# ccuchengwei/LongReadSelfCorrect

Hardware: AMD Instinct MI355X
Metric: corrected Mbases/s (whole node) (higher is better)
Workload: dtype int64

## Files before the change

longreadselfcorrect_amd/csrc/capi_batch.cpp:

```cpp
#include <cmath>
#include <limits>

#include "capi_internal.h"

using namespace lrsc;

extern "C" void lrsc_batch_destroy(lrsc_batch* b)
{
    if(!b) return;
    if(b->ctx) (void)hipSetDevice(b->ctx->device);
    if(b->d_codes) (void)hipFree(b->d_codes);
    if(b->d_off) (void)hipFree(b->d_off);
    if(b->d_chunk) (void)hipFree(b->d_chunk);
    void* ptrs[] = {b->d_freq, b->d_base_counted, b->d_valid, b->d_flags, b->d_zeros, b->d_attr, b->d_start_bits, b->d_seeds,
                    b->d_seed_count, b->d_thr, b->d_scan_tmp, b->d_outcasts, b->d_outcast_count, b->d_walk_log, b->d_ratio};
    for(void* q : ptrs) if(q) (void)hipFree(q);
    delete b;
}

extern "C" int lrsc_batch_create(lrsc_ctx* ctx, const char* reads, const uint64_t* read_off, uint32_t n_reads,
                                 lrsc_batch** out)
{
    if(!ctx || !out || n_reads == 0) return fail(LRSC_ERR_ARG, "null / empty batch");
    int st = check_offsets(read_off, n_reads);
    if(st != LRSC_OK) return st;
    const uint64_t total = read_off[n_reads];
    if(total == 0 || !reads) return fail(LRSC_ERR_ARG, "empty batch");
    HIP_TRY(hipSetDevice(ctx->device));
    lrsc_batch* b = new(std::nothrow) lrsc_batch();
    if(!b) return fail(LRSC_ERR_NOMEM, "lrsc_batch");
    b->ctx = ctx;
    b->n_reads = n_reads;
    b->total_bases = total;
    const uint64_t n_chunks = (total + (1ull << kChunkShift) - 1) >> kChunkShift;
    hipError_t e = hipMalloc(reinterpret_cast<void**>(&b->d_codes), total);
    if(e == hipSuccess) e = hipMalloc(reinterpret_cast<void**>(&b->d_off), (n_reads + 1) * sizeof(uint64_t));
    if(e == hipSuccess) e = hipMalloc(reinterpret_cast<void**>(&b->d_chunk), n_chunks * sizeof(uint32_t));
    if(e != hipSuccess) { lrsc_batch_destroy(b); return hip_fail(e, "batch alloc"); }
    const uint64_t slice = 256ull << 20;
    for(uint64_t o = 0; o < total; o += slice) {
        const uint64_t n = std::min(slice, total - o);
        st = upload_and_encode(ctx, reads + o, n, b->d_codes + o);
        if(st != LRSC_OK) { lrsc_batch_destroy(b); return st; }
    }
    e = hipMemcpyAsync(b->d_off, read_off, (n_reads + 1) * sizeof(uint64_t), hipMemcpyHostToDevice, ctx->stream);
    if(e == hipSuccess) e = launch_chunk_table(b->d_off, n_reads, total, b->d_chunk, ctx->stream);
    if(e == hipSuccess) e = hipStreamSynchronize(ctx->stream);
    if(e != hipSuccess) { lrsc_batch_destroy(b); return hip_fail(e, "batch upload"); }
    *out = b;
    return LRSC_OK;
}

static uint32_t pool_from_params(const lrsc_params& p, uint8_t* ks)
{
    std::vector<int> v = {5, 9, p.scan_kmer_len};
    for(int i = 0; i < 3; ++i) v.push_back(p.start_kmer_len + p.offset[i]);
    std::sort(v.begin(), v.end());
    v.erase(std::unique(v.begin(), v.end()), v.end());
    uint32_t n = 0;
    for(int x : v) if(x > 0 && x < 256 && n < kMaxPool) ks[n++] = (uint8_t)x;
    return n;
}

static const float kThresholdFormula[3][6] = {
    {0.0004799107143, -0.008037815126, 0.03673552754, 0.1850695903, -1.572552521, 18.0522088},
    {0.0003348214286, -0.009112394958, 0.04286714686, 0.240519958, -1.8793367350, 21.29319228},
    {0.01714285714, -0.6193907563, 2.266956783, 17.28450630, -100.6983493, 1103.571729}};

extern "C" int lrsc_kmer_thresholds_range(int coverage, int end, float* out)
{
    if(!out || end < 15) return fail(LRSC_ERR_ARG, "null table / end < 15");
    const int start = 15, stride = end + 2;
    for(int mode = 0; mode < 3; ++mode) {
        for(int k = 0; k < stride; ++k) out[mode * stride + k] = 0.0f;
        float cavity = std::numeric_limits<float>::max();
        const float* f = kThresholdFormula[mode];
        const int x = coverage;
        for(int y = start; y <= end; ++y) {
            float v = f[0] * x * x + f[1] * x * y + f[2] * y * y + f[3] * x + f[4] * y + f[5];
            v = std::fmax(v, 2.0f);
            cavity = std::fmin(cavity, v);
            out[mode * stride + y] = cavity;
        }
    }
    return LRSC_OK;
}

extern "C" int lrsc_kmer_thresholds(int coverage, float* out)
{
    return lrsc_kmer_thresholds_range(coverage, 50, out);
}

static int batch_setup_rows(lrsc_ctx* ctx, lrsc_batch* b)
{
    if(b->n_k != 0) return LRSC_OK;
    const lrsc_params& p = ctx->params;
    b->n_k = pool_from_params(p, b->ks);
    for(auto& x : b->row_of_k) x = -1;
    for(auto& x : b->freq_index) x = -1;
    int wanted[4] = {p.scan_kmer_len, p.start_kmer_len + p.offset[0], p.start_kmer_len + p.offset[1],
                     p.start_kmer_len + p.offset[2]};
    int min_k = 1 << 30;
    for(int i = 0; i < 4; ++i) {
        const int k = wanted[i];
        if(k <= 0 || k > 51) return fail(LRSC_ERR_ARG, "k-mer sizes must lie in 1..51");
        if(i > 0 && k < min_k) min_k = k;
        if(b->row_of_k[k] >= 0) continue;
        for(uint32_t j = 0; j < b->n_k; ++j)
            if(b->ks[j] == k) { b->freq_index[j] = (int8_t)b->n_rows; b->row_of_k[k] = (int8_t)b->n_rows; ++b->n_rows; }
        if(b->row_of_k[k] < 0) return fail(LRSC_ERR_ARG, "k-mer size missing from the pool");
    }
    b->min_k = (uint32_t)min_k;
    if(b->total_bases >= (1ull << 32)) return fail(LRSC_ERR_UNSUPPORTED, "a resident batch holds < 2^32 bases");
    HIP_TRY(hipMalloc(reinterpret_cast<void**>(&b->d_freq), (size_t)b->n_rows * b->total_bases * sizeof(int32_t)));
    HIP_TRY(hipMalloc(reinterpret_cast<void**>(&b->d_base_counted), b->total_bases));
    HIP_TRY(hipMalloc(reinterpret_cast<void**>(&b->d_valid), b->total_bases));
    return LRSC_OK;
}

static GridArgs batch_grid_args(const lrsc_batch* b)
{
    GridArgs a{};
    a.codes = b->d_codes;
    a.read_off = b->d_off;
    a.chunk_read = b->d_chunk;
    a.total_bases = b->total_bases;
    a.n_reads = b->n_reads;
    a.n_k = b->n_k;
    for(uint32_t i = 0; i < b->n_k; ++i) { a.ks[i] = b->ks[i]; a.freq_index[i] = b->freq_index[i]; }
    a.freq = b->d_freq;
    a.base_counted = b->d_base_counted;
    a.valid_mask = b->d_valid;
    return a;
}

extern "C" int lrsc_batch_kmer_grid(lrsc_ctx* ctx, lrsc_batch* b)
{
    if(!ctx || !b || b->ctx != ctx) return fail(LRSC_ERR_ARG, "batch does not belong to this ctx");
    HIP_TRY(hipSetDevice(ctx->device));
    int st = batch_setup_rows(ctx, b);
    if(st != LRSC_OK) return st;
    const GridArgs a = batch_grid_args(b);
    st = timed_launch(ctx, LRSC_K_GRID, [&]() { return launch_kmer_grid(ctx->fm, a, ctx->d_ctr, ctx->stream); });
    if(st == LRSC_OK) b->grid_done = true;
    return st;
}

static int batch_setup_seeds(lrsc_ctx* ctx, lrsc_batch* b)
{
    if(b->d_seeds) return LRSC_OK;
    b->seed_cap = b->total_bases / b->min_k + b->n_reads + 1;
    HIP_TRY(hipMalloc(reinterpret_cast<void**>(&b->d_flags), b->total_bases * sizeof(unsigned long long)));
    HIP_TRY(hipMalloc(reinterpret_cast<void**>(&b->d_zeros), b->total_bases * sizeof(uint32_t)));
    HIP_TRY(hipMalloc(reinterpret_cast<void**>(&b->d_attr), b->total_bases));
    HIP_TRY(hipMalloc(reinterpret_cast<void**>(&b->d_start_bits), ((b->total_bases + 255) / 256) * 4 * sizeof(unsigned long long)));
    HIP_TRY(hipMalloc(reinterpret_cast<void**>(&b->d_seeds), b->seed_cap * kSeedInts * sizeof(int32_t)));
    HIP_TRY(hipMalloc(reinterpret_cast<void**>(&b->d_seed_count), (size_t)b->n_reads * sizeof(uint32_t)));
    if(b->debug_flags & LRSC_DEBUG_RATIO) HIP_TRY(hipMalloc(reinterpret_cast<void**>(&b->d_ratio), b->total_bases * sizeof(float)));
    if(b->debug_flags & LRSC_DEBUG_OUTCASTS) {
        HIP_TRY(hipMalloc(reinterpret_cast<void**>(&b->d_outcasts), b->seed_cap * kSeedInts * sizeof(int32_t)));
        HIP_TRY(hipMalloc(reinterpret_cast<void**>(&b->d_outcast_count), (size_t)b->n_reads * sizeof(uint32_t)));
    }
    HIP_TRY(hipMalloc(reinterpret_cast<void**>(&b->d_thr), 3 * 52 * sizeof(float)));
    float thr[3 * 52];
    (void)lrsc_kmer_thresholds(ctx->params.pb_coverage, thr);
    HIP_TRY(hipMemcpy(b->d_thr, thr, sizeof(thr), hipMemcpyHostToDevice));
    return LRSC_OK;
}

static SeedArgs batch_seed_args(const lrsc_ctx* ctx, const lrsc_batch* b)
{
    const lrsc_params& p = ctx->params;
    SeedArgs a{};
    a.codes = b->d_codes; a.read_off = b->d_off; a.chunk_read = b->d_chunk;
    a.total_bases = b->total_bases; a.n_reads = b->n_reads;
    a.freq = b->d_freq; a.valid_mask = b->d_valid; a.base_counted = b->d_base_counted;
    for(int i = 0; i < 64; ++i) a.row_of_k[i] = b->row_of_k[i];
    a.base_k = b->ks[0];
    a.start_kmer_len = p.start_kmer_len; a.scan_kmer_len = p.scan_kmer_len; a.kmer_len_up_bound = p.kmer_len_up_bound;
    a.pb_coverage = p.pb_coverage; a.mode = p.mode; a.manual = p.manual; a.radius = p.radius;
    for(int i = 0; i < 3; ++i) a.offset[i] = p.offset[i];
    a.hh_ratio = p.hh_ratio;
    a.thresholds = b->d_thr;
    a.flags = b->d_flags; a.zeros = b->d_zeros; a.attribute = b->d_attr; a.start_bits = b->d_start_bits; a.seeds = b->d_seeds; a.seed_count = b->d_seed_count;
    a.outcasts = b->d_outcasts; a.outcast_count = b->d_outcast_count; a.ratio = b->d_ratio;
    return a;
}

extern "C" int lrsc_batch_find_seeds(lrsc_ctx* ctx, lrsc_batch* b)
{
    if(!ctx || !b || b->ctx != ctx) return fail(LRSC_ERR_ARG, "batch does not belong to this ctx");
    if(ctx->params.kmer_len_up_bound > 50) return fail(LRSC_ERR_ARG, "kmer_len_up_bound must be <= 50 (threshold table)");
    if(ctx->params.manual && (ctx->params.mode < 0 || ctx->params.mode > 2)) return fail(LRSC_ERR_ARG, "mode must be 0, 1 or 2");
    int st = lrsc_batch_kmer_grid(ctx, b);
    if(st != LRSC_OK) return st;
    st = batch_setup_seeds(ctx, b);
    if(st != LRSC_OK) return st;
    const SeedArgs a = batch_seed_args(ctx, b);
    st = timed_launch(ctx, LRSC_K_SEEDS, [&]() {
        hipError_t e = launch_seed_modes(a, ctx->stream);
        if(e == hipSuccess) e = scan_seed_flags(b->d_flags, b->d_zeros, b->total_bases, &b->d_scan_tmp, &b->scan_tmp_cap, ctx->stream);
        if(e == hipSuccess) e = launch_seed_attribute(a, ctx->stream);
        if(e == hipSuccess) e = launch_seed_scan(ctx->fm, a, b->min_k, ctx->d_ctr, ctx->stream);
        return e;
    });
    if(st == LRSC_OK) b->seeds_done = true;
    return st;
}

extern "C" int lrsc_batch_seeds(lrsc_ctx* ctx, lrsc_batch* b, uint32_t* seed_count, lrsc_seed* seeds, uint64_t cap,
                                uint64_t* n_seeds, int8_t* attribute)
{
    if(!ctx || !b || b->ctx != ctx || !seed_count || !n_seeds) return fail(LRSC_ERR_ARG, "null / foreign batch");
    if(!b->seeds_done) return fail(LRSC_ERR_ARG, "call lrsc_batch_find_seeds first");
    HIP_TRY(hipSetDevice(ctx->device));
    HIP_TRY(hipMemcpy(seed_count, b->d_seed_count, (size_t)b->n_reads * sizeof(uint32_t), hipMemcpyDeviceToHost));
    std::vector<uint64_t> off(b->n_reads + 1);
    HIP_TRY(hipMemcpy(off.data(), b->d_off, off.size() * sizeof(uint64_t), hipMemcpyDeviceToHost));
    uint64_t total = 0;
    for(uint32_t r = 0; r < b->n_reads; ++r) total += seed_count[r];
    *n_seeds = total;
    if(total > cap) return fail(LRSC_ERR_CAPACITY, "seed buffer too small");
    if(seeds) {
        static_assert(sizeof(lrsc_seed) == kSeedInts * sizeof(int32_t), "lrsc_seed layout");
        uint64_t w = 0;
        for(uint32_t r = 0; r < b->n_reads; ++r) {
            if(seed_count[r] == 0) continue;
            const uint64_t slab = seed_slab(off[r], r, b->min_k);
            HIP_TRY(hipMemcpy(seeds + w, b->d_seeds + slab * kSeedInts, (size_t)seed_count[r] * sizeof(lrsc_seed),
                              hipMemcpyDeviceToHost));
            w += seed_count[r];
        }
    }
    if(attribute) HIP_TRY(hipMemcpy(attribute, b->d_attr, b->total_bases, hipMemcpyDeviceToHost));
    return LRSC_OK;
}

extern "C" int lrsc_find_seeds(lrsc_ctx* ctx, const char* reads, const uint64_t* read_off, uint32_t n_reads,
                               uint32_t* seed_count, lrsc_seed* seeds, uint64_t cap, uint64_t* n_seeds, int8_t* attribute)
{
    lrsc_batch* b = nullptr;
    int st = lrsc_batch_create(ctx, reads, read_off, n_reads, &b);
    if(st != LRSC_OK) return st;
    st = lrsc_batch_find_seeds(ctx, b);
    if(st == LRSC_OK) st = lrsc_batch_seeds(ctx, b, seed_count, seeds, cap, n_seeds, attribute);
    lrsc_batch_destroy(b);
    return st;
}

extern "C" int lrsc_batch_set_debug(lrsc_batch* b, int flags)
{
    if(!b) return fail(LRSC_ERR_ARG, "null batch");
    if(flags & ~(LRSC_DEBUG_OUTCASTS | LRSC_DEBUG_WALKS | LRSC_DEBUG_RATIO)) return fail(LRSC_ERR_ARG, "unknown debug flag");
    if(b->d_seeds) return fail(LRSC_ERR_ARG, "lrsc_batch_set_debug must precede lrsc_batch_find_seeds");
    b->debug_flags = flags;
    return LRSC_OK;
}

extern "C" int lrsc_batch_outcast_seeds(lrsc_ctx* ctx, lrsc_batch* b, uint32_t* outcast_count, lrsc_seed* seeds, uint64_t cap,
                                        uint64_t* n_seeds)
{
    if(!ctx || !b || b->ctx != ctx || !outcast_count || !n_seeds) return fail(LRSC_ERR_ARG, "null / foreign batch");
    if(!b->seeds_done || !b->d_outcasts) return fail(LRSC_ERR_ARG, "needs LRSC_DEBUG_OUTCASTS and lrsc_batch_find_seeds");
    HIP_TRY(hipSetDevice(ctx->device));
    HIP_TRY(hipMemcpy(outcast_count, b->d_outcast_count, (size_t)b->n_reads * sizeof(uint32_t), hipMemcpyDeviceToHost));
    std::vector<uint64_t> off(b->n_reads + 1);
    HIP_TRY(hipMemcpy(off.data(), b->d_off, off.size() * sizeof(uint64_t), hipMemcpyDeviceToHost));
    uint64_t total = 0;
    for(uint32_t r = 0; r < b->n_reads; ++r) total += outcast_count[r];
    *n_seeds = total;
    if(total > cap) return fail(LRSC_ERR_CAPACITY, "seed buffer too small");
    uint64_t w = 0;
    for(uint32_t r = 0; seeds && r < b->n_reads; ++r) {
        if(outcast_count[r] == 0) continue;
        const uint64_t slab = seed_slab(off[r], r, b->min_k);
        HIP_TRY(hipMemcpy(seeds + w, b->d_outcasts + slab * kSeedInts, (size_t)outcast_count[r] * sizeof(lrsc_seed), hipMemcpyDeviceToHost));
        w += outcast_count[r];
    }
    return LRSC_OK;
}

extern "C" int lrsc_batch_repeat_ratio(lrsc_ctx* ctx, lrsc_batch* b, float* ratio)
{
    if(!ctx || !b || b->ctx != ctx || !ratio) return fail(LRSC_ERR_ARG, "null / foreign batch");
    if(!b->seeds_done || !b->d_ratio) return fail(LRSC_ERR_ARG, "needs LRSC_DEBUG_RATIO and lrsc_batch_find_seeds");
    HIP_TRY(hipSetDevice(ctx->device));
    HIP_TRY(hipMemcpy(ratio, b->d_ratio, b->total_bases * sizeof(float), hipMemcpyDeviceToHost));
    return LRSC_OK;
}

extern "C" int lrsc_batch_walk_log(lrsc_ctx* ctx, lrsc_batch* b, uint8_t* log, uint64_t cap)
{
    if(!ctx || !b || b->ctx != ctx || !log) return fail(LRSC_ERR_ARG, "null / foreign batch");
    if(!b->walk_log_done || !b->d_walk_log) return fail(LRSC_ERR_ARG, "needs LRSC_DEBUG_WALKS and lrsc_batch_correct");
    HIP_TRY(hipSetDevice(ctx->device));
    std::vector<uint32_t> count(b->n_reads);
    std::vector<uint64_t> off(b->n_reads + 1);
    HIP_TRY(hipMemcpy(count.data(), b->d_seed_count, count.size() * sizeof(uint32_t), hipMemcpyDeviceToHost));
    HIP_TRY(hipMemcpy(off.data(), b->d_off, off.size() * sizeof(uint64_t), hipMemcpyDeviceToHost));
    std::vector<uint8_t> all(b->seed_cap);
    HIP_TRY(hipMemcpy(all.data(), b->d_walk_log, b->seed_cap, hipMemcpyDeviceToHost));
    uint64_t w = 0;
    for(uint32_t r = 0; r < b->n_reads; ++r) {
        if(w + count[r] > cap) return fail(LRSC_ERR_CAPACITY, "walk log buffer too small");
        if(count[r]) std::memcpy(log + w, all.data() + seed_slab(off[r], r, b->min_k), count[r]);
        w += count[r];
    }
    return LRSC_OK;
}
```

longreadselfcorrect_amd/csrc/capi_core.cpp:

```cpp
#include <cmath>
#include <limits>

#include "capi_internal.h"

using namespace lrsc;

static thread_local std::string g_last_error;

int lrsc::fail(int status, const std::string& msg)
{
    g_last_error = msg;
    return status;
}
int lrsc::hip_fail(hipError_t e, const char* what)
{
    g_last_error = std::string(what) + ": " + hipGetErrorString(e);
    return LRSC_ERR_DEVICE;
}

extern "C" const char* lrsc_strerror(int status)
{
    switch(status) {
        case LRSC_OK: return "ok";
        case LRSC_ERR_IO: return "I/O error";
        case LRSC_ERR_FORMAT: return "BWT file is not properly formatted";
        case LRSC_ERR_ARG: return "invalid argument";
        case LRSC_ERR_NOMEM: return "out of memory";
        case LRSC_ERR_DEVICE: return "HIP device error";
        case LRSC_ERR_CAPACITY: return "output buffer too small";
        case LRSC_ERR_UNSUPPORTED: return "unsupported";
        case LRSC_ERR_LIMIT: return "internal capacity exceeded";
        default: return "unknown error";
    }
}
extern "C" const char* lrsc_last_error(void) { return g_last_error.c_str(); }
extern "C" int lrsc_abi_version(void) { return LRSC_ABI_VERSION; }

extern "C" int lrsc_params_default(int genome, int coverage, lrsc_params* out)
{
    if(!out) return fail(LRSC_ERR_ARG, "null params");
    int order;
    switch(genome) {
        case 5: order = 0; break;
        case 10: order = 1; break;
        case 100: order = 2; break;
        default: return fail(LRSC_ERR_ARG, "genome must be 5, 10 or 100");
    }
    static const int size[3] = {17, 19, 21};
    std::memset(out, 0, sizeof(*out));
    out->pb_coverage = coverage;
    out->error_rate = 0.15;
    out->start_kmer_len = size[order];
    out->offset[0] = 0;
    out->offset[1] = 2 * std::min(std::max(coverage / 30 - 1, 0), order + 1);
    out->offset[2] = -2 * (order + 1);
    out->mode = 1;
    out->manual = 0;
    out->scan_kmer_len = 19;
    out->kmer_len_up_bound = 50;
    out->radius = 100;
    out->hh_ratio = 0.6f;
    out->next_target = 1;
    out->max_leaves = 32;
    out->idmer_len = 9;
    out->min_kmer_len = 13;
    out->split = 0;
    out->no_dp = 0;
    return LRSC_OK;
}

uint64_t lrsc::env_bytes(const char* name, uint64_t dflt, unsigned shift)
{
    if(const char* e = std::getenv(name)) return std::max<uint64_t>(1, (uint64_t)std::atoll(e)) << shift;
    return dflt;
}

static uint32_t env_clamped(const char* name, uint32_t dflt, int lo, int hi)
{
    if(const char* e = std::getenv(name)) return (uint32_t)std::min(hi, std::max(lo, std::atoi(e)));
    return dflt;
}

uint32_t lrsc::resident_waves(const lrsc_ctx* ctx, uint32_t per_simd)
{
    int cus = 256;
    (void)hipDeviceGetAttribute(&cus, hipDeviceAttributeMultiprocessorCount, ctx->device);
    return (uint32_t)cus * 4u * per_simd;
}

Tunables lrsc::read_tunables(const lrsc_ctx* ctx)
{
    const int kIntMax = std::numeric_limits<int>::max();
    Tunables t;
    t.wp_prep_bytes = env_bytes("LRSC_WP_PREP_MB", 24ull << 30, 20);
    t.wp_lane_bytes = env_bytes("LRSC_WP_LANE_MB", 32ull << 30, 20);
    t.wp_lanes = env_clamped("LRSC_WP_LANES", resident_waves(ctx, 2) * 64u, 64, kIntMax);
    t.wp_gen_quorum = env_clamped("LRSC_WP_GEN_QUORUM", 70, 0, 100);
    t.wp_gen_wait = env_clamped("LRSC_WP_GEN_WAIT", 6, 0, kIntMax);
    t.wp_wide_cap = env_clamped("LRSC_WP_WIDE_CAP", kNarrowLeaves, 1, (int)kNarrowLeaves);
    t.wp_wave = env_clamped("LRSC_WP_WAVE", 1, 0, 2);
    { const char* e = std::getenv("LRSC_WP_BEGIN_SORT"); t.wp_begin_sort = e && e[0] != '0'; }
    t.dp_chunk_bytes = env_bytes("LRSC_DP_CHUNK_MB", 16ull << 30, 20);
    t.dp_align_waves = env_clamped("LRSC_DP_ALIGN_WAVES", 0, 0, kIntMax);
    t.msa_force_global = std::getenv("LRSC_MSA_FORCE_GLOBAL") != nullptr;
    { const char* e = std::getenv("LRSC_MSA_BATCH"); t.msa_batch = !(e && e[0] == '0'); }
    t.profile = std::getenv("LRSC_CORRECT_PROFILE") != nullptr;
    t.wp_dump = std::getenv("LRSC_WP_DUMP") != nullptr;
    t.dp_debug = std::getenv("LRSC_DP_DEBUG") != nullptr;
    return t;
}

int lrsc::check_offsets(const uint64_t* off, uint32_t n_reads)
{
    if(!off) return fail(LRSC_ERR_ARG, "null read offsets");
    if(off[0] != 0) return fail(LRSC_ERR_ARG, "read_off[0] must be 0");
    for(uint32_t i = 0; i < n_reads; ++i)
        if(off[i + 1] < off[i]) return fail(LRSC_ERR_ARG, "read offsets must be non-decreasing");
    return LRSC_OK;
}

static const char* const kMaxLeavesMsg = "max_leaves must be 1..256";
static_assert(kWideMaxLeaves == 256, "kMaxLeavesMsg names the cap");

int lrsc::check_walk_params(const lrsc_params& p)
{
    if(p.max_leaves < 1 || p.max_leaves > (int)kWideMaxLeaves) return fail(LRSC_ERR_UNSUPPORTED, kMaxLeavesMsg);
    if(p.idmer_len < 5 || p.idmer_len > 16) return fail(LRSC_ERR_UNSUPPORTED, "idmer_len must be 5..16");
    if(p.min_kmer_len < p.idmer_len || p.min_kmer_len > 62) return fail(LRSC_ERR_UNSUPPORTED, "min_kmer_len out of range");
    return LRSC_OK;
}

void lrsc::kmer_freq_table(const lrsc_params& p, double freqs[101])
{
    for(int i = 0; i <= 100; ++i) freqs[i] = 0;
    for(int i = p.min_kmer_len; i <= 100; i++) freqs[i] = pow(1 - p.error_rate, i) * (size_t)p.pb_coverage;
}

int lrsc::encode_acgt(const char* seq, uint64_t n, uint8_t* codes)
{
    for(uint64_t i = 0; i < n; ++i) {
        switch(seq[i]) {
            case 'A': codes[i] = 0; break; case 'C': codes[i] = 1; break; case 'G': codes[i] = 2; break; case 'T': codes[i] = 3; break;
            default: return fail(LRSC_ERR_ARG, "sequence contains a base other than A,C,G,T");
        }
    }
    return LRSC_OK;
}

int lrsc::upload_and_encode(lrsc_ctx* ctx, const char* ascii, uint64_t n, uint8_t* d_codes)
{
    HIP_TRY(ctx->s_in.reserve(n));
    HIP_TRY(ctx->s_flag.reserve(1));
    HIP_TRY(hipMemsetAsync(ctx->s_flag.p, 0, sizeof(int), ctx->stream));
    HIP_TRY(hipMemcpyAsync(ctx->s_in.p, ascii, n, hipMemcpyHostToDevice, ctx->stream));
    hipError_t e = launch_encode(reinterpret_cast<const char*>(ctx->s_in.p), d_codes, n, ctx->s_flag.p, ctx->stream);
    if(e != hipSuccess) return hip_fail(e, "encode");
    int bad = 0;
    HIP_TRY(hipMemcpyAsync(&bad, ctx->s_flag.p, sizeof(int), hipMemcpyDeviceToHost, ctx->stream));
    HIP_TRY(hipStreamSynchronize(ctx->stream));
    if(bad) return fail(LRSC_ERR_ARG, "sequence contains a base other than A,C,G,T");
    return LRSC_OK;
}

int lrsc::stage_reads(lrsc_ctx* ctx, const char* tool, unsigned limit_log2, const char* reads, const uint64_t* read_off, uint32_t n_reads, uint64_t slack)
{
    const int st = check_offsets(read_off, n_reads);
    if(st != LRSC_OK) return st;
    for(uint32_t i = 0; i < n_reads; ++i) {
        const uint64_t len = read_off[i + 1] - read_off[i];
        if(len == 0) return fail(LRSC_ERR_ARG, std::string(tool) + ": read " + std::to_string(i) + " is empty");
        if(len >> limit_log2) return fail(LRSC_ERR_UNSUPPORTED, std::string(tool) + ": a read of 2^" + std::to_string(limit_log2) + " bases or more");
    }
    const uint64_t total = read_off[n_reads];
    HIP_TRY(hipSetDevice(ctx->device));
    HIP_TRY(ctx->s_codes.reserve(total + slack));
    HIP_TRY(ctx->s_off.reserve((uint64_t)n_reads + 1));
    const int enc = upload_and_encode(ctx, reads, total, ctx->s_codes.p);
    if(enc != LRSC_OK) return enc;
    HIP_TRY(hipMemcpyAsync(ctx->s_off.p, read_off, ((uint64_t)n_reads + 1) * sizeof(uint64_t), hipMemcpyHostToDevice, ctx->stream));
    HIP_TRY(hipMemsetAsync(ctx->s_flag.p, 0, sizeof(int), ctx->stream));
    return LRSC_OK;
}

extern "C" int lrsc_ctx_create(const lrsc_index* idx, const lrsc_params* params, int device, lrsc_ctx** out)
{
    if(!idx || !out) return fail(LRSC_ERR_ARG, "null");
    lrsc_index* midx = const_cast<lrsc_index*>(idx);
    FmIndexDev fm;
    {
        std::lock_guard<std::mutex> lock(midx->mu);
        auto it = midx->copies.find(device);
        if(it == midx->copies.end()) return fail(LRSC_ERR_DEVICE, "index not uploaded to this device (call lrsc_index_upload)");
        fm = it->second.dev;
    }
    HIP_TRY(hipSetDevice(device));
    lrsc_ctx* ctx = new(std::nothrow) lrsc_ctx();
    if(!ctx) return fail(LRSC_ERR_NOMEM, "lrsc_ctx");
    ctx->index = idx;
    ctx->device = device;
    ctx->fm = fm;
    if(params) ctx->params = *params;
    else (void)lrsc_params_default(10, 90, &ctx->params);
    hipError_t e = hipStreamCreateWithFlags(&ctx->stream, hipStreamNonBlocking);
    if(e == hipSuccess) e = hipEventCreate(&ctx->ev0);
    if(e == hipSuccess) e = hipEventCreate(&ctx->ev1);
    if(e == hipSuccess) e = hipMalloc(reinterpret_cast<void**>(&ctx->d_ctr), kCtrShards * sizeof(DevCounters));
    if(e == hipSuccess) e = hipMemset(ctx->d_ctr, 0, kCtrShards * sizeof(DevCounters));
    if(e != hipSuccess) { lrsc_ctx_destroy(ctx); return hip_fail(e, "lrsc_ctx_create"); }
    *out = ctx;
    return LRSC_OK;
}

extern "C" void lrsc_ctx_destroy(lrsc_ctx* ctx) { delete ctx; }

extern "C" int lrsc_ctx_get_params(const lrsc_ctx* ctx, lrsc_params* out)
{
    if(!ctx || !out) return fail(LRSC_ERR_ARG, "null");
    *out = ctx->params;
    return LRSC_OK;
}

extern "C" int lrsc_ctx_sync(lrsc_ctx* ctx)
{
    if(!ctx) return fail(LRSC_ERR_ARG, "null ctx");
    HIP_TRY(hipSetDevice(ctx->device));
    HIP_TRY(hipStreamSynchronize(ctx->stream));
    return LRSC_OK;
}

extern "C" int lrsc_ctx_stats(lrsc_ctx* ctx, int kernel, lrsc_kernel_stats* out)
{
    if(!ctx || !out || kernel < 0 || kernel >= LRSC_K_COUNT) return fail(LRSC_ERR_ARG, "bad stats query");
    *out = ctx->stats[kernel];
    return LRSC_OK;
}
extern "C" int lrsc_ctx_stats_reset(lrsc_ctx* ctx)
{
    if(!ctx) return fail(LRSC_ERR_ARG, "null ctx");
    for(auto& s : ctx->stats) s = lrsc_kernel_stats{};
    return LRSC_OK;
}
```

longreadselfcorrect_amd/csrc/capi_correct.cpp:

```cpp
#include "capi_internal.h"

using namespace lrsc;

struct lrsc::CorrectScratch {
    DevBuf<ReadPlan> d_plan;
    DevBuf<uint32_t> d_pieces;
    DevBuf<uint8_t> d_codes_out;
    DevBuf<uint64_t> d_dst_off;
    DevBuf<char> d_dst;
    DevBuf<double> d_freqs;
    DpStage stage;
    DevBuf<WpReadWork> d_work;
    DevBuf<WpRead> d_reads;
    DevBuf<WpSlot> d_slots;
    DevBuf<uint64_t> d_sz;
    DevBuf<uint32_t> d_key, d_key_tmp, d_list, d_list_tmp;
    DevBuf<uint32_t> d_small;
    DevBuf<WpDpItem> d_items, d_items2, d_items3;
    DevBuf<DevCounters> d_ctr2;
    hipEvent_t ev_side_t0 = nullptr, ev_side_t1 = nullptr;
    DevBuf<WpRequest> d_req;
    DevBuf<uint8_t> d_prep, d_lane, d_lane_side, d_lane_wide;
    DevBuf<uint32_t> d_wide_list;
    DevBuf<uint32_t> d_sort9;
    hipStream_t side = nullptr;
    hipEvent_t ev_ready = nullptr;
    DevBuf<unsigned long long> d_prof;
    DevArena persist;
    void* cub_tmp = nullptr;
    size_t cub_cap = 0;
    ~CorrectScratch()
    {
        if(cub_tmp) (void)hipFree(cub_tmp);
        if(side) { (void)hipStreamSynchronize(side); (void)hipStreamDestroy(side); }
        if(ev_ready) (void)hipEventDestroy(ev_ready);
        if(ev_side_t0) (void)hipEventDestroy(ev_side_t0);
        if(ev_side_t1) (void)hipEventDestroy(ev_side_t1);
    }
};

lrsc_ctx::~lrsc_ctx()
{
    (void)hipSetDevice(device);
    if(stream) (void)hipStreamSynchronize(stream);
    delete cs;
    if(d_ctr) (void)hipFree(d_ctr);
    if(ev0) (void)hipEventDestroy(ev0);
    if(ev1) (void)hipEventDestroy(ev1);
    if(stream) (void)hipStreamDestroy(stream);
}

namespace {

static_assert(sizeof(WpRequest) == 2 * sizeof(uint32_t), "WpRequest records are staged in a uint32_t buffer");

struct WpFlow {
    lrsc_ctx* const ctx;
    lrsc_batch* const b;
    CorrectScratch& sc;
    const lrsc_params& p;
    const Tunables tn;
    const uint32_t n;
    const uint32_t lbytes;
    const bool escalate;
    WpArgs a{};
    std::vector<ReadPlan> plan;
    std::vector<uint32_t> seed_count;
    std::vector<uint64_t> off;
    std::vector<WpReadWork> work;
    std::vector<int> skipped;
    uint64_t out_total = 0, piece_total = 0, n_slots = 0;
    uint32_t r0 = 0, r1 = 0, n_range = 0;
    uint64_t slot_base = 0;
    std::vector<WpDpItem> items;
    std::vector<DpRequest> reqs;
    std::vector<WpRequest> hreq;
    std::vector<uint32_t> hlist;
    uint64_t n_escalated = 0;

    struct Round {
        uint32_t index = 0;
        uint32_t n_ent = 0;
        uint64_t tot[3] = {};
        uint32_t stats[4] = {};
        const uint32_t* ext_list = nullptr;
        uint32_t n_mid = 0;
        bool long_launch = false;
        bool long_pending = false;
        uint32_t n_items = 0;
        unsigned long long begin_stats[4] = {};
    };

    WpFlow(lrsc_ctx* ctx_, lrsc_batch* b_)
        : ctx(ctx_), b(b_), sc(*ctx_->cs), p(ctx_->params), tn(read_tunables(ctx_)), n(b_->n_reads),
          lbytes((uint32_t)leaf_bytes(ctx_->fm.wide != 0)), escalate((uint32_t)ctx_->params.max_leaves > tn.wp_wide_cap)
    {
    }

    uint32_t* small(WpSmall word) const { return sc.d_small.p + word; }

    int bounds_and_slots();
    int bind_args();
    void choose_range(uint32_t first);
    int run_range();
    int gather_results(lrsc_read_result* res, uint64_t* piece_off, uint64_t piece_cap, char* out, uint64_t out_cap,
                       uint64_t* n_pieces_out, uint64_t* out_used);
    int print_extension_profile();

    int round_entries(Round& R, bool* done);
    int plan_and_materialise(Round& R);
    int launch_order(Round& R);
    int extension_launches(Round& R);
    int escalate_walks(const WpArgs& x0, uint32_t n_ent, uint32_t pathw);
    int start_long_walks(Round& R);
    int dp_calls(Round& R);
    int finish_long_walks();
    int stitch();
    int dump_range_walks();
    void print_round(const Round& R) const;

    hipError_t extend_range(WpArgs x, const uint32_t* list, const WpRequest* rq, uint32_t count, uint32_t pathw, hipStream_t st,
                            bool side, uint32_t stride);
    int fetch_items(DevBuf<WpDpItem>& d_list, const uint32_t* d_count, uint32_t cap, Round& R, std::vector<WpDpItem>& out);
    int dp_call(std::vector<WpDpItem>& its);
};

int WpFlow::bounds_and_slots()
{
    double freqs[101];
    kmer_freq_table(p, freqs);
    HIP_TRY(sc.d_plan.reserve(n));
    HIP_TRY(sc.d_freqs.reserve(101));
    HIP_TRY(hipMemcpyAsync(sc.d_freqs.p, freqs, sizeof(freqs), hipMemcpyHostToDevice, ctx->stream));

    WpArgs pa{};
    pa.codes = b->d_codes; pa.read_off = b->d_off; pa.seeds = b->d_seeds; pa.seed_count = b->d_seed_count;
    pa.n_reads = n; pa.min_k = b->min_k; pa.next_target = p.next_target;
    hipError_t e = launch_wp_bounds(pa, sc.d_plan.p, ctx->stream);
    if(e != hipSuccess) return hip_fail(e, "wp_bounds");
    plan.resize(n); seed_count.resize(n); off.resize(n + 1);
    HIP_TRY(hipMemcpyAsync(plan.data(), sc.d_plan.p, (size_t)n * sizeof(ReadPlan), hipMemcpyDeviceToHost, ctx->stream));
    HIP_TRY(hipMemcpyAsync(seed_count.data(), b->d_seed_count, (size_t)n * sizeof(uint32_t), hipMemcpyDeviceToHost, ctx->stream));
    HIP_TRY(hipMemcpyAsync(off.data(), b->d_off, (size_t)(n + 1) * sizeof(uint64_t), hipMemcpyDeviceToHost, ctx->stream));
    HIP_TRY(hipStreamSynchronize(ctx->stream));

    work.resize(n);
    skipped.assign(n, 0);
    for(uint32_t r = 0; r < n; ++r) {
        WpReadWork& w = work[r];
        std::memset(&w, 0, sizeof(w));
        const uint64_t rlen = off[r + 1] - off[r];
        const uint32_t ns = seed_count[r];
        w.out_off = out_total; w.piece_off = piece_total; w.slot_first = n_slots;
        if(ns < 2) continue;
        const uint64_t cap = rlen + (uint64_t)((p.no_dp ? 1.2 : 2.0) * (double)rlen) + (uint64_t)ns * (2 * kMaxInitK + 16 + (p.no_dp ? 0 : 128)) + 64;
        if(cap >= (1ull << 32)) { skipped[r] = LRSC_READ_TOO_LONG; continue; }
        if(plan[r].lq_max >= 65535) { skipped[r] = LRSC_READ_WALK_QUERY_TOO_LONG; continue; }
        w.out_cap = (uint32_t)cap;
        w.piece_cap = p.split ? ns : 1;
        w.n_seeds = ns;
        out_total += ((uint64_t)w.out_cap + 15) & ~15ull;
        piece_total += w.piece_cap;
        n_slots += ns - 1;
    }
    if(n_slots >= (1ull << 32)) return fail(LRSC_ERR_UNSUPPORTED, "batch: more than 2^32 seed pairs (split the input)");

    HIP_TRY(sc.d_work.reserve(n));
    HIP_TRY(sc.d_reads.reserve(n));
    HIP_TRY(sc.d_slots.reserve(std::max<uint64_t>(n_slots, 1)));
    HIP_TRY(sc.d_small.reserve(kWpSmallWords));
    HIP_TRY(sc.d_req.reserve(n));
    HIP_TRY(sc.d_codes_out.reserve(std::max<uint64_t>(out_total, 64)));
    HIP_TRY(sc.d_pieces.reserve(std::max<uint64_t>(piece_total, 1)));
    HIP_TRY(hipMemcpyAsync(sc.d_work.p, work.data(), (size_t)n * sizeof(WpReadWork), hipMemcpyHostToDevice, ctx->stream));
    HIP_TRY(hipMemsetAsync(sc.d_reads.p, 0, (size_t)n * sizeof(WpRead), ctx->stream));
    return LRSC_OK;
}

int WpFlow::bind_args()
{
    a.codes = b->d_codes; a.read_off = b->d_off; a.seeds = b->d_seeds; a.seed_count = b->d_seed_count;
    a.n_reads = n; a.min_k = b->min_k;
    a.work = sc.d_work.p; a.reads = sc.d_reads.p; a.slots = sc.d_slots.p; a.n_slots = n_slots;
    a.seed_size = (uint32_t)p.idmer_len; a.min_overlap = (uint32_t)p.min_kmer_len; a.max_leaves = (uint32_t)p.max_leaves;
    if(escalate) { a.max_leaves = tn.wp_wide_cap; a.escalate = 1; }
    a.start_kmer_len = p.start_kmer_len; a.next_target = p.next_target; a.split = p.split; a.no_dp = p.no_dp;
    a.pb_coverage = (uint64_t)p.pb_coverage; a.pacbio_error_rate = p.error_rate;
    a.freqs_of_kmer_size = sc.d_freqs.p;
    a.psz = ctx->fm.wide ? 8 : 4; a.lbytes = lbytes;
    a.plan_stats = small(kWpSmallPlanStats); a.queue = small(kWpSmallQueue); a.n_dp_items = small(kWpSmallDpItems);
    a.n_req_out = small(kWpSmallReqOut);
    a.n_sort9 = small(kWpSmallSort9); a.begin_sort = tn.wp_begin_sort ? 1u : 0u;
    a.req_out = sc.d_req.p; a.req_cap = n;
    a.out_codes = sc.d_codes_out.p; a.piece_start = sc.d_pieces.p;
    a.auto_dp = (!p.no_dp && p.next_target == 1) ? 1u : 0u;
    a.general_quorum_pct = tn.wp_gen_quorum; a.general_max_wait = tn.wp_gen_wait;
    a.ctr = ctx->d_ctr;
    if(b->debug_flags & LRSC_DEBUG_WALKS) {
        if(!b->d_walk_log) HIP_TRY(hipMalloc(reinterpret_cast<void**>(&b->d_walk_log), b->seed_cap));
        HIP_TRY(hipMemsetAsync(b->d_walk_log, 0, b->seed_cap, ctx->stream));
        a.walk_log = b->d_walk_log;
        b->walk_log_done = false;
    }
    if(tn.profile) {
        HIP_TRY(sc.d_prof.reserve(36));
        HIP_TRY(hipMemsetAsync(sc.d_prof.p, 0, 36 * sizeof(unsigned long long), ctx->stream));
        a.prof = sc.d_prof.p;
        a.begin_stats = sc.d_prof.p + 32;
    }
    if(!sc.side) HIP_TRY(hipStreamCreateWithFlags(&sc.side, hipStreamNonBlocking));
    if(!sc.ev_ready) HIP_TRY(hipEventCreateWithFlags(&sc.ev_ready, hipEventDisableTiming));
    return LRSC_OK;
}

void WpFlow::choose_range(uint32_t first)
{
    r0 = r1 = first;
    uint64_t est = 0;
    while(r1 < n) {
        const uint64_t ns = work[r1].n_seeds;
        const uint64_t need = ns >= 2 ? 55 * (off[r1 + 1] - off[r1]) + ns * 4400 : 0;
        if(r1 > r0 && est + need > tn.wp_prep_bytes) break;
        est += need;
        ++r1;
    }
    slot_base = work[r0].slot_first;
    const uint64_t slot_end = r1 < n ? work[r1].slot_first : n_slots;
    n_range = (uint32_t)(slot_end - slot_base);
    a.r0 = r0; a.r1 = r1; a.slot_base = slot_base;
}

int WpFlow::run_range()
{
    sc.persist.reset();
    if(n_range == 0) return LRSC_OK;
    for(uint32_t round = 0;; ++round) {
        Round R;
        R.index = round;
        bool done = false;
        int st = round_entries(R, &done);
        if(st != LRSC_OK) return st;
        if(done) break;
        st = plan_and_materialise(R);
        if(st == LRSC_OK) st = launch_order(R);
        if(st == LRSC_OK) st = extension_launches(R);
        if(st == LRSC_OK && escalate) st = escalate_walks(a, R.n_ent, std::max(R.stats[2], 1u));
        if(st == LRSC_OK && R.long_launch) st = start_long_walks(R);
        if(st == LRSC_OK) st = dp_calls(R);
        if(st == LRSC_OK) st = stitch();
        if(st == LRSC_OK && tn.profile && round == 0 && tn.wp_dump) st = dump_range_walks();
        if(st != LRSC_OK) return st;
        if(tn.profile) {
            HIP_TRY(hipStreamSynchronize(ctx->stream));
            HIP_TRY(hipMemcpy(R.begin_stats, a.begin_stats, sizeof(R.begin_stats), hipMemcpyDeviceToHost));
            print_round(R);
        }
        if(round > 100000) return fail(LRSC_ERR_LIMIT, "walk-parallel flow: too many rounds");
    }
    return LRSC_OK;
}

int WpFlow::round_entries(Round& R, bool* done)
{
    uint32_t n_ent = n_range;
    a.list = nullptr; a.reqs = nullptr;
    if(R.index != 0) {
        uint32_t n_req = 0;
        HIP_TRY(hipStreamSynchronize(ctx->stream));
        HIP_TRY(hipMemcpy(&n_req, a.n_req_out, sizeof(uint32_t), hipMemcpyDeviceToHost));
        if(n_req == 0) { *done = true; return LRSC_OK; }
        if(n_req > n) return fail(LRSC_ERR_LIMIT, "walk-parallel flow: request list overflow");
        hreq.resize(n_req);
        HIP_TRY(hipMemcpy(hreq.data(), sc.d_req.p, (size_t)n_req * sizeof(WpRequest), hipMemcpyDeviceToHost));
        std::sort(hreq.begin(), hreq.end(), [](const WpRequest& x, const WpRequest& y) { return x.slot < y.slot; });
        hlist.resize(n_req);
        for(uint32_t i = 0; i < n_req; ++i) hlist[i] = hreq[i].slot;
        n_ent = n_req;
    }
    R.n_ent = n_ent;
    HIP_TRY(sc.d_sz.reserve(3 * ((size_t)n_ent + 1)));
    HIP_TRY(sc.d_key.reserve(n_ent));
    HIP_TRY(sc.d_key_tmp.reserve(n_ent));
    HIP_TRY(sc.d_list.reserve(n_ent));
    HIP_TRY(sc.d_list_tmp.reserve(n_ent));
    HIP_TRY(sc.d_items.reserve(n_ent));
    HIP_TRY(sc.d_sort9.reserve(2 * (size_t)n_ent));
    a.sort9 = sc.d_sort9.p;
    if(a.begin_stats) HIP_TRY(hipMemsetAsync(a.begin_stats, 0, 4 * sizeof(unsigned long long), ctx->stream));
    a.sz_q = sc.d_sz.p; a.sz_prep = sc.d_sz.p + (n_ent + 1); a.sz_path = sc.d_sz.p + 2 * ((size_t)n_ent + 1);
    a.sort_key = sc.d_key.p;
    a.n_list = n_ent;
    a.dp_items = sc.d_items.p; a.dp_items_cap = n_ent;
    HIP_TRY(hipMemsetAsync(sc.d_sz.p, 0, 3 * ((size_t)n_ent + 1) * sizeof(uint64_t), ctx->stream));
    HIP_TRY(hipMemsetAsync(sc.d_small.p, 0, kWpSmallWords * sizeof(uint32_t), ctx->stream));
    if(R.index != 0) {
        HIP_TRY(sc.d_list_tmp.reserve(2 * (size_t)n_ent));
        WpRequest* d_reqs_in = reinterpret_cast<WpRequest*>(sc.d_list_tmp.p);
        HIP_TRY(hipMemcpyAsync(d_reqs_in, hreq.data(), (size_t)n_ent * sizeof(WpRequest), hipMemcpyHostToDevice, ctx->stream));
        HIP_TRY(hipMemcpyAsync(sc.d_list.p, hlist.data(), (size_t)n_ent * sizeof(uint32_t), hipMemcpyHostToDevice, ctx->stream));
        a.list = sc.d_list.p; a.reqs = d_reqs_in;
    }
    return LRSC_OK;
}

int WpFlow::plan_and_materialise(Round& R)
{
    const uint32_t n_ent = R.n_ent;
    hipError_t e = launch_wp_plan(a, ctx->stream);
    if(e != hipSuccess) return hip_fail(e, "wp_plan");
    for(int j = 0; j < 3; ++j) {
        e = wp_scan(sc.d_sz.p + (size_t)j * (n_ent + 1), (uint64_t)n_ent + 1, &sc.cub_tmp, &sc.cub_cap, ctx->stream);
        if(e != hipSuccess) return hip_fail(e, "wp_scan");
    }
    for(int j = 0; j < 3; ++j)
        HIP_TRY(hipMemcpyAsync(&R.tot[j], sc.d_sz.p + (size_t)j * (n_ent + 1) + n_ent, sizeof(uint64_t), hipMemcpyDeviceToHost, ctx->stream));
    HIP_TRY(hipMemcpyAsync(R.stats, small(kWpSmallPlanStats), sizeof(R.stats), hipMemcpyDeviceToHost, ctx->stream));
    HIP_TRY(hipStreamSynchronize(ctx->stream));
    HIP_TRY(sc.persist.alloc(R.tot[0] + 64, &a.arena_q));
    HIP_TRY(sc.persist.alloc(R.tot[2] + 64, &a.arena_path));
    HIP_TRY(sc.d_prep.reserve(R.tot[1] + 64));
    a.arena_prep = sc.d_prep.p;
    e = launch_wp_materialize(a, ctx->stream);
    if(e != hipSuccess) return hip_fail(e, "wp_materialize");
    return LRSC_OK;
}

int WpFlow::launch_order(Round& R)
{
    R.ext_list = a.list;
    if(R.index != 0) return LRSC_OK;
    hlist.resize(R.n_ent);
    for(uint32_t i = 0; i < R.n_ent; ++i) hlist[i] = (uint32_t)slot_base + i;
    HIP_TRY(hipMemcpyAsync(sc.d_list_tmp.p, hlist.data(), (size_t)R.n_ent * sizeof(uint32_t), hipMemcpyHostToDevice, ctx->stream));
    hipError_t e = wp_sort_list(sc.d_key.p, sc.d_key_tmp.p, sc.d_list.p, sc.d_list_tmp.p, R.n_ent, &sc.cub_tmp, &sc.cub_cap, ctx->stream);
    if(e != hipSuccess) return hip_fail(e, "wp_sort_list");
    R.ext_list = sc.d_list.p;
    R.n_mid = R.stats[0];
    return LRSC_OK;
}

hipError_t WpFlow::extend_range(WpArgs x, const uint32_t* list, const WpRequest* rq, uint32_t count, uint32_t pathw, hipStream_t st,
                                bool side, uint32_t stride)
{
    if(count == 0) return hipSuccess;
    if(tn.wp_wave == 2) stride = 64;
    const WpLaneLayout LL = wp_lane_layout(lbytes, pathw);
    const uint64_t slots = tn.wp_lanes / 64;
    const uint64_t share = side ? std::max<uint64_t>(1, slots / 2) : slots;
    uint64_t lanes = std::min<uint64_t>(stride == 1 ? (((uint64_t)count + 63) & ~63ull) : count, share * 64 / stride);
    lanes = std::max<uint64_t>(1, std::min<uint64_t>(lanes, (tn.wp_lane_bytes / (side ? 4 : 1)) / LL.total));
    if(stride == 1) lanes = std::max<uint64_t>(64, lanes & ~63ull);
    DevBuf<uint8_t>& buf = side ? sc.d_lane_side : sc.d_lane;
    hipError_t e = buf.reserve(lanes * LL.total);
    if(e != hipSuccess) return e;
    x.list = list; x.reqs = rq; x.n_list = count;
    x.lane_ws = buf.p; x.lane_ws_bytes = LL.total; x.lane_pathw = pathw; x.n_lanes = (uint32_t)lanes; x.lane_stride = stride;
    x.queue = small(side ? kWpSmallSideQueue : kWpSmallExtQueue);
    e = hipMemsetAsync(x.queue, 0, sizeof(uint32_t), st);
    if(e != hipSuccess) return e;
    if(stride == 64 && tn.wp_wave != 0) return launch_wp_extend_wave(ctx->fm, x, st);
    return launch_wp_extend(ctx->fm, x, st);
}

int WpFlow::extension_launches(Round& R)
{
    return timed_launch(ctx, LRSC_K_EXTEND, [&]() -> hipError_t {
        hipError_t e = launch_wp_prepare(ctx->fm, a, ctx->stream);
        if(e == hipSuccess) e = launch_wp_begin(ctx->fm, a, ctx->stream);
        if(e != hipSuccess) return e;
        if(R.index != 0)
            return extend_range(a, a.list, a.reqs, R.n_ent, std::max(R.stats[2], 1u), ctx->stream, false,
                                R.n_ent <= 16384 ? 64u : R.n_ent <= 65536 ? 16u : 1u);
        e = extend_range(a, R.ext_list + R.n_mid, nullptr, R.n_ent - R.n_mid, std::min(R.stats[2], kWpPathwSmall), ctx->stream, false, 1);
        if(e != hipSuccess || R.n_mid == 0) return e;
        if(p.no_dp || escalate) return extend_range(a, R.ext_list, nullptr, R.n_mid, R.stats[2], ctx->stream, false, 64);
        R.long_launch = true;
        return e;
    });
}

int WpFlow::escalate_walks(const WpArgs& x0, uint32_t n_ent, uint32_t pathw)
{
    HIP_TRY(sc.d_wide_list.reserve(n_ent));
    uint32_t* d_count = small(kWpSmallWideCount);
    HIP_TRY(hipMemsetAsync(d_count, 0, sizeof(uint32_t), ctx->stream));
    hipError_t e = launch_wp_wide_collect(x0, sc.d_wide_list.p, d_count, ctx->stream);
    if(e != hipSuccess) return hip_fail(e, "wp_wide_collect");
    uint32_t n_wide = 0;
    HIP_TRY(hipMemcpyAsync(&n_wide, d_count, sizeof(uint32_t), hipMemcpyDeviceToHost, ctx->stream));
    HIP_TRY(hipStreamSynchronize(ctx->stream));
    if(n_wide > n_ent) return fail(LRSC_ERR_LIMIT, "walk-parallel flow: escalation list overflow");
    n_escalated += n_wide;
    if(n_wide == 0) return LRSC_OK;
    WpArgs x = x0;
    x.max_leaves = (uint32_t)p.max_leaves; x.escalate = 0;
    x.list = sc.d_wide_list.p; x.reqs = nullptr; x.n_list = n_wide;
    const WpWideLayout WL = wp_wide_layout(lbytes, pathw, x.max_leaves);
    uint64_t waves = std::min<uint64_t>(n_wide, tn.wp_lanes / 64);
    waves = std::max<uint64_t>(1, std::min<uint64_t>(waves, (tn.wp_lane_bytes / 4) / WL.total));
    HIP_TRY(sc.d_lane_wide.reserve(waves * WL.total));
    x.lane_ws = sc.d_lane_wide.p; x.lane_ws_bytes = WL.total; x.lane_pathw = pathw; x.n_lanes = (uint32_t)waves; x.lane_stride = 64;
    x.queue = small(kWpSmallWideQueue);
    HIP_TRY(hipMemsetAsync(x.queue, 0, sizeof(uint32_t), ctx->stream));
    return timed_launch(ctx, LRSC_K_EXTEND_WIDE, [&]() { return launch_wp_extend_wide(ctx->fm, x, ctx->stream); });
}

int WpFlow::start_long_walks(Round& R)
{
    HIP_TRY(sc.d_items2.reserve(R.n_mid));
    WpArgs xl = a;
    xl.dp_items = sc.d_items2.p; xl.n_dp_items = small(kWpSmallSideDpItems); xl.dp_items_cap = R.n_mid;
    HIP_TRY(sc.d_ctr2.reserve(kCtrShards));
    HIP_TRY(hipMemsetAsync(sc.d_ctr2.p, 0, kCtrShards * sizeof(DevCounters), ctx->stream));
    xl.ctr = sc.d_ctr2.p;
    if(a.prof) xl.prof = a.prof + 16;
    HIP_TRY(hipEventRecord(sc.ev_ready, ctx->stream));
    HIP_TRY(hipStreamWaitEvent(sc.side, sc.ev_ready, 0));
    if(!sc.ev_side_t0) HIP_TRY(hipEventCreate(&sc.ev_side_t0));
    HIP_TRY(hipEventRecord(sc.ev_side_t0, sc.side));
    hipError_t e = extend_range(xl, R.ext_list, nullptr, R.n_mid, R.stats[2], sc.side, true, 64);
    if(e != hipSuccess) return hip_fail(e, "wp_extend (long walks)");
    R.long_pending = true;
    return LRSC_OK;
}

int WpFlow::fetch_items(DevBuf<WpDpItem>& d_list, const uint32_t* d_count, uint32_t cap, Round& R, std::vector<WpDpItem>& out)
{
    uint32_t cnt = 0;
    HIP_TRY(hipMemcpy(&cnt, d_count, sizeof(uint32_t), hipMemcpyDeviceToHost));
    if(cnt > cap) return fail(LRSC_ERR_LIMIT, "walk-parallel flow: DP item list overflow");
    R.n_items += cnt;
    out.resize(cnt);
    if(cnt) HIP_TRY(hipMemcpy(out.data(), d_list.p, (size_t)cnt * sizeof(WpDpItem), hipMemcpyDeviceToHost));
    std::sort(out.begin(), out.end(), [](const WpDpItem& x, const WpDpItem& y) { return x.slot < y.slot; });
    return LRSC_OK;
}

int WpFlow::dp_call(std::vector<WpDpItem>& its)
{
    const uint32_t cnt = (uint32_t)its.size();
    if(cnt == 0) return LRSC_OK;
    reqs.clear();
    reqs.reserve(cnt);
    for(const WpDpItem& it : its) {
        DpRequest q;
        std::memset(&q, 0, sizeof(q));
        q.q_off = it.q;
        q.lq = it.lq; q.k = it.k;
        q.coverage = (uint32_t)p.pb_coverage;
        q.min_overlap = it.lq / 10;
        const size_t total = (size_t)it.total_freq;
        double identity = 0.65;
        size_t min_call_coverage = 15;
        identity += (total > 50 ? 0.05 : 0);
        identity += (total > 100 ? 0.05 : 0);
        min_call_coverage = total > 50 ? total * 0.4 : min_call_coverage;
        q.min_identity = identity; q.min_call_coverage = (int32_t)min_call_coverage;
        reqs.push_back(q);
    }
    const int sd = sc.stage.run(ctx, tn, nullptr, reqs);
    if(sd != LRSC_OK) return sd;
    uint8_t* cons_keep = nullptr;
    HIP_TRY(sc.persist.alloc(sc.stage.cons_total + 64, &cons_keep));
    HIP_TRY(hipMemcpyAsync(cons_keep, sc.stage.d_cons.p, sc.stage.cons_total, hipMemcpyDeviceToDevice, ctx->stream));
    HIP_TRY(sc.d_items3.reserve(cnt));
    HIP_TRY(hipMemcpyAsync(sc.d_items3.p, its.data(), (size_t)cnt * sizeof(WpDpItem), hipMemcpyHostToDevice, ctx->stream));
    WpArgs c2 = a;
    c2.dp_reqs = sc.stage.d_reqs.p; c2.dp_msa = sc.stage.d_msa.p; c2.dp_cons = cons_keep; c2.n_dp = cnt;
    hipError_t ec = launch_wp_dp_collect(c2, sc.d_items3.p, ctx->stream);
    if(ec != hipSuccess) return hip_fail(ec, "wp_dp_collect");
    HIP_TRY(hipStreamSynchronize(ctx->stream));
    return LRSC_OK;
}

int WpFlow::finish_long_walks()
{
    if(!sc.ev_side_t1) HIP_TRY(hipEventCreate(&sc.ev_side_t1));
    HIP_TRY(hipEventRecord(sc.ev_side_t1, sc.side));
    HIP_TRY(hipEventSynchronize(sc.ev_side_t1));
    float ms = 0.f;
    HIP_TRY(hipEventElapsedTime(&ms, sc.ev_side_t0, sc.ev_side_t1));
    lrsc_kernel_stats& s = ctx->stats[LRSC_K_EXTEND];
    s.total_ms += ms;
    std::vector<DevCounters> shards(kCtrShards);
    HIP_TRY(hipMemcpy(shards.data(), sc.d_ctr2.p, kCtrShards * sizeof(DevCounters), hipMemcpyDeviceToHost));
    for(const DevCounters& dcn : shards) {
        s.rank_queries += dcn.rank_queries;
        s.block_loads += dcn.block_loads;
        s.table_loads += dcn.table_loads;
    }
    return LRSC_OK;
}

int WpFlow::dp_calls(Round& R)
{
    int sd = fetch_items(sc.d_items, a.n_dp_items, R.n_ent, R, items);
    if(sd != LRSC_OK) return sd;
    sd = dp_call(items);
    if(sd != LRSC_OK || !R.long_pending) return sd;
    sd = finish_long_walks();
    if(sd != LRSC_OK) return sd;
    std::vector<WpDpItem> longs;
    sd = fetch_items(sc.d_items2, small(kWpSmallSideDpItems), R.n_mid, R, longs);
    if(sd != LRSC_OK) return sd;
    return dp_call(longs);
}

int WpFlow::stitch()
{
    HIP_TRY(hipMemsetAsync(a.n_req_out, 0, sizeof(uint32_t), ctx->stream));
    hipError_t e = launch_wp_stitch(a, ctx->stream);
    if(e != hipSuccess) return hip_fail(e, "wp_stitch");
    return LRSC_OK;
}

int WpFlow::dump_range_walks()
{
    std::vector<WpSlot> hs(n_range);
    HIP_TRY(hipStreamSynchronize(ctx->stream));
    HIP_TRY(hipMemcpy(hs.data(), sc.d_slots.p + slot_base, (size_t)n_range * sizeof(WpSlot), hipMemcpyDeviceToHost));
    std::vector<uint32_t> ord(n_range);
    for(uint32_t i = 0; i < n_range; ++i) ord[i] = i;
    std::sort(ord.begin(), ord.end(), [&](uint32_t x, uint32_t y) { return hs[x].leaf_steps > hs[y].leaf_steps; });
    unsigned long long tot = 0, tot_steps = 0;
    for(const WpSlot& q : hs) { tot += q.leaf_steps; tot_steps += q.steps; }
    std::fprintf(stderr, "[lrsc] wp walks of the range: %u, %llu steps, %llu leaf-steps; hardest (gap, k, steps, leaf-steps, code):", n_range, tot_steps, tot);
    for(uint32_t i = 0; i < std::min<uint32_t>(n_range, 12); ++i)
        std::fprintf(stderr, " (%u,%u,%u,%u,%d)", hs[ord[i]].gap, (unsigned)hs[ord[i]].k, hs[ord[i]].steps, hs[ord[i]].leaf_steps, hs[ord[i]].code);
    unsigned long long hist[34] = {0}, wsteps[34] = {0};
    for(const WpSlot& q : hs) { const unsigned m = std::min<unsigned>(q.max_front, 33); hist[m]++; wsteps[m] += q.leaf_steps; }
    std::fprintf(stderr, "; walks (and their leaf-steps in %%) by widest frontier:");
    for(unsigned m = 1; m < 34; ++m)
        if(hist[m]) std::fprintf(stderr, " %u:%.2f%%(%.1f%%)", m, 100.0 * hist[m] / n_range, 100.0 * wsteps[m] / std::max(tot, 1ull));
    const uint32_t qs[] = {n_range / 2, n_range / 10, n_range / 100, n_range / 1000, n_range / 10000};
    std::fprintf(stderr, "; leaf-steps at the median / top 10%% / 1%% / 0.1%% / 0.01%%: %u %u %u %u %u\n", hs[ord[qs[0]]].leaf_steps, hs[ord[qs[1]]].leaf_steps,
                 hs[ord[qs[2]]].leaf_steps, hs[ord[qs[3]]].leaf_steps, hs[ord[qs[4]]].leaf_steps);
    return LRSC_OK;
}

void WpFlow::print_round(const Round& R) const
{
    std::fprintf(stderr, "[lrsc] wp reads [%u, %u) round %u: %u entries, %u DP requests (%llu strings), arenas q %.1f MB prep %.1f MB path %.1f MB, %llu walks escalated so far\n",
                 r0, r1, R.index, R.n_ent, R.n_items, (unsigned long long)sc.stage.n_strings, R.tot[0] / 1048576.0, R.tot[1] / 1048576.0, R.tot[2] / 1048576.0,
                 (unsigned long long)n_escalated);
    const unsigned long long* g = R.begin_stats;
    if(tn.wp_begin_sort)
        std::fprintf(stderr, "[lrsc] wp reads [%u, %u) round %u: wp_begin %llu interval lists, %llu entries, every list sorted (LRSC_WP_BEGIN_SORT)\n",
                     r0, r1, R.index, g[0], g[2] + g[3]);
    else
        std::fprintf(stderr, "[lrsc] wp reads [%u, %u) round %u: wp_begin %llu interval lists, %llu with a repeated code (%.1f%%); entries %llu in the lists without one, %llu in those with one\n",
                     r0, r1, R.index, g[0], g[1], 100.0 * g[1] / std::max(g[0], 1ull), g[2], g[3]);
}

int WpFlow::print_extension_profile()
{
    unsigned long long prs[32];
    HIP_TRY(hipStreamSynchronize(ctx->stream));
    HIP_TRY(hipStreamSynchronize(sc.side));
    HIP_TRY(hipMemcpy(prs, sc.d_prof.p, sizeof(prs), hipMemcpyDeviceToHost));
    for(int part = 0; part < 2; ++part) {
        const unsigned long long* pr = prs + 16 * part;
        if(pr[10] == 0) continue;
        const double all = (double)pr[10], st = (double)std::max<unsigned long long>(pr[11], 1);
        std::fprintf(stderr, "[lrsc] wp extension kernel (%s), lane wall ticks: %.3g total, %.0f per step over %.3g steps; extendLeaves %.1f%% (refine %.1f%%, attempToExtend %.1f%% of which "
                             "getFMIndexExtensions %.1f%%), PrunedBySeedSupport %.1f%%, materialise+commit %.1f%%, isTerminated %.1f%%, refill %.1f%%, finish %.1f%%; single-leaf fast steps %.1f%% of the steps in %.1f%% of the ticks\n",
                     part ? "long-gap walks, one per wavefront" : "bulk and later rounds",
                     all, all / st, st, 100 * pr[0] / all, 100 * pr[1] / all, 100 * pr[2] / all, 100 * pr[3] / all, 100 * pr[4] / all, 100 * pr[5] / all, 100 * pr[6] / all,
                     100 * pr[8] / all, 100 * pr[9] / all, 100 * pr[12] / st, 100 * pr[7] / all);
    }
    return LRSC_OK;
}

int WpFlow::gather_results(lrsc_read_result* res, uint64_t* piece_off, uint64_t piece_cap, char* out, uint64_t out_cap,
                           uint64_t* n_pieces_out, uint64_t* out_used)
{
    std::vector<WpRead> ro(n);
    HIP_TRY(hipStreamSynchronize(ctx->stream));
    HIP_TRY(hipMemcpy(ro.data(), sc.d_reads.p, (size_t)n * sizeof(WpRead), hipMemcpyDeviceToHost));
    std::vector<uint32_t> pieces(std::max<uint64_t>(piece_total, 1));
    if(piece_total) HIP_TRY(hipMemcpy(pieces.data(), sc.d_pieces.p, (size_t)piece_total * sizeof(uint32_t), hipMemcpyDeviceToHost));
    std::vector<uint64_t> dst_off(n + 1, 0);
    uint64_t n_pieces = 0;
    for(uint32_t r = 0; r < n; ++r) {
        const WpRead& o = ro[r];
        int status = skipped[r];
        if(o.error == LRSC_WALK_ERR_GEOMETRY) status = LRSC_READ_GEOMETRY;
        else if(o.error == LRSC_WALK_ERR_CODE) status = LRSC_READ_INTERNAL;
        else if(o.error == LRSC_WALK_ERR_DP) status = LRSC_READ_DP_LIMIT;
        else if(o.error == LRSC_WALK_ERR_OUTPUT) status = LRSC_READ_OUTPUT_LIMIT;
        else if(o.error != 0) status = LRSC_READ_FRONTIER_LIMIT;
        lrsc_read_result& R = res[r];
        if(status != LRSC_READ_OK) {
            std::memset(&R, 0, sizeof(R));
            R.piece_first = n_pieces;
            R.status = status;
            dst_off[r + 1] = dst_off[r];
            continue;
        }
        R.merge = (int32_t)o.merge; R.n_pieces = o.n_pieces; R.piece_first = n_pieces;
        R.total_reads_len = (int64_t)(off[r + 1] - off[r]); R.corrected_len = o.c[1]; R.total_seed_num = seed_count[r]; R.total_walk_num = o.c[3];
        R.high_error_num = o.c[4]; R.exceed_depth_num = o.c[5]; R.exceed_leave_num = o.c[6]; R.fm_num = o.c[7];
        R.dp_num = o.c[8]; R.seed_dis = o.c[9];
        R.status = LRSC_READ_OK; R.pad = 0;
        dst_off[r + 1] = dst_off[r] + o.out_len;
        for(uint32_t j = 0; j < o.n_pieces; ++j) {
            if(piece_off && n_pieces < piece_cap) piece_off[n_pieces] = dst_off[r] + pieces[work[r].piece_off + j];
            ++n_pieces;
        }
    }
    const uint64_t used = dst_off[n];
    if(piece_off && n_pieces < piece_cap) piece_off[n_pieces] = used;
    *n_pieces_out = n_pieces;
    *out_used = used;
    if(!out || !piece_off || used > out_cap || n_pieces + 1 > piece_cap) return fail(LRSC_ERR_CAPACITY, "output buffers too small");
    if(used) {
        HIP_TRY(sc.d_dst_off.reserve(n + 1));
        HIP_TRY(sc.d_dst.reserve(used));
        HIP_TRY(hipMemcpyAsync(sc.d_dst_off.p, dst_off.data(), (size_t)(n + 1) * sizeof(uint64_t), hipMemcpyHostToDevice, ctx->stream));
        hipError_t e = launch_wp_gather(a, sc.d_dst_off.p, sc.d_dst.p, ctx->stream);
        if(e != hipSuccess) return hip_fail(e, "wp_gather");
        HIP_TRY(hipMemcpyAsync(out, sc.d_dst.p, used, hipMemcpyDeviceToHost, ctx->stream));
        HIP_TRY(hipStreamSynchronize(ctx->stream));
    }
    return LRSC_OK;
}

int batch_correct_wp(lrsc_ctx* ctx, lrsc_batch* b, lrsc_read_result* res, uint64_t* piece_off, uint64_t piece_cap, char* out,
                     uint64_t out_cap, uint64_t* n_pieces_out, uint64_t* out_used)
{
    if(!ctx->cs) ctx->cs = new(std::nothrow) CorrectScratch();
    if(!ctx->cs) return fail(LRSC_ERR_NOMEM, "correct scratch");
    WpFlow f(ctx, b);
    int st = f.bounds_and_slots();
    if(st == LRSC_OK) st = f.bind_args();
    for(uint32_t first = 0; st == LRSC_OK && first < f.n; first = f.r1) {
        f.choose_range(first);
        st = f.run_range();
    }
    if(st == LRSC_OK && f.a.prof) st = f.print_extension_profile();
    if(st != LRSC_OK) return st;
    if(f.a.walk_log) b->walk_log_done = true;
    return f.gather_results(res, piece_off, piece_cap, out, out_cap, n_pieces_out, out_used);
}

}

extern "C" int lrsc_batch_correct(lrsc_ctx* ctx, lrsc_batch* b, lrsc_read_result* res, uint64_t* piece_off, uint64_t piece_cap,
                                  char* out, uint64_t out_cap, uint64_t* n_pieces_out, uint64_t* out_used)
{
    if(!ctx || !b || b->ctx != ctx || !res || !n_pieces_out || !out_used) return fail(LRSC_ERR_ARG, "null / foreign batch");
    *n_pieces_out = 0; *out_used = 0;
    const lrsc_params& p = ctx->params;
    int st = check_walk_params(p);
    if(st != LRSC_OK) return st;
    if(p.next_target < 1) return fail(LRSC_ERR_ARG, "next_target must be >= 1");
    const uint32_t n = b->n_reads;
    if(n == 0) return LRSC_OK;
    HIP_TRY(hipSetDevice(ctx->device));
    if(!b->seeds_done) {
        st = lrsc_batch_find_seeds(ctx, b);
        if(st != LRSC_OK) return st;
    }
    return batch_correct_wp(ctx, b, res, piece_off, piece_cap, out, out_cap, n_pieces_out, out_used);
}
```

longreadselfcorrect_amd/csrc/capi_dp.cpp:

```cpp
#include "capi_internal.h"

using namespace lrsc;

struct DpAlignClasses {
    struct Class { uint32_t max_s1 = 0, stage_max = 0; uint64_t jobs = 0; } cls[kDpAlignClasses + 1];
    std::vector<DpOrderRun> runs;
    DpOrder order;
    void add(uint32_t s1_len, uint32_t stage_bytes, uint32_t first_job, uint32_t n_jobs)
    {
        const uint32_t k = dp_align_class(stage_bytes);
        Class& c = cls[k];
        c.max_s1 = std::max(c.max_s1, s1_len); c.stage_max = std::max(c.stage_max, stage_bytes); c.jobs += n_jobs;
        if(n_jobs) runs.push_back({k, first_job, n_jobs});
    }
    void sort() { order = dp_order_build(runs); }
    uint32_t waves(uint32_t k, uint32_t lds_waves, uint32_t wave_cap) const
    {
        const Class& c = cls[k];
        if(!c.jobs) return 0;
        uint64_t want = k < kDpAlignClasses ? lds_waves : 1024;
        if(wave_cap) want = std::min<uint64_t>(want, wave_cap);
        const uint64_t stride = (uint64_t)(c.max_s1 + 17) * kDpTraceStride;
        return (uint32_t)std::max<uint64_t>(1, std::min<uint64_t>(std::min<uint64_t>(want, c.jobs), (4ull << 30) / stride));
    }
    int upload(lrsc_ctx* ctx, DevBuf<uint32_t>& d_order, DevBuf<uint32_t>& d_heads) const
    {
        HIP_TRY(d_order.reserve(std::max<size_t>(order.list.size(), 1)));
        HIP_TRY(d_heads.reserve(kDpAlignClasses + 1));
        if(!order.list.empty())
            HIP_TRY(hipMemcpyAsync(d_order.p, order.list.data(), order.list.size() * sizeof(uint32_t), hipMemcpyHostToDevice, ctx->stream));
        HIP_TRY(hipMemsetAsync(d_heads.p, 0, (kDpAlignClasses + 1) * sizeof(uint32_t), ctx->stream));
        return LRSC_OK;
    }
    int launch(lrsc_ctx* ctx, DpAlignArgs al, uint32_t lds_waves, uint32_t wave_cap, DevBuf<uint8_t>& d_trace, DevBuf<uint8_t>& d_seq_ws,
               const DevBuf<uint32_t>& d_order, const DevBuf<uint32_t>& d_heads) const
    {
        uint32_t nw[kDpAlignClasses + 1] = {};
        uint64_t stride[kDpAlignClasses + 1] = {}, trace_bytes = 0, ws_bytes = 0;
        for(uint32_t k = 0; k <= kDpAlignClasses; ++k) {
            const Class& c = cls[k];
            if(!c.jobs) continue;
            stride[k] = (uint64_t)(c.max_s1 + 17) * kDpTraceStride;
            nw[k] = waves(k, lds_waves, wave_cap);
            trace_bytes = std::max(trace_bytes, stride[k] * nw[k]);
            if(k == kDpAlignClasses) ws_bytes = (((uint64_t)c.stage_max + 255) & ~255ull) * nw[k];
        }
        HIP_TRY(d_trace.reserve(std::max<uint64_t>(trace_bytes, 64)));
        if(ws_bytes) HIP_TRY(d_seq_ws.reserve(ws_bytes));
        al.trace = d_trace.p;
        for(uint32_t k = 0; k <= kDpAlignClasses; ++k) {
            if(!nw[k]) continue;
            if(order.size(k) != cls[k].jobs) return fail(LRSC_ERR_DEVICE, "dp_align: a class's job list does not hold its jobs");
            al.list = d_order.p + order.begin[k]; al.n_list = order.size(k); al.head = d_heads.p + k;
            al.stage_max = cls[k].stage_max;
            al.trace_stride = stride[k];
            al.seq_ws = k < kDpAlignClasses ? nullptr : d_seq_ws.p;
            al.seq_ws_stride = k < kDpAlignClasses ? 0 : ((uint64_t)cls[k].stage_max + 255) & ~255ull;
            const uint32_t n = nw[k];
            const int st = timed_launch(ctx, LRSC_K_DP, [&]() { return launch_dp_align(al, n, ctx->stream); });
            if(st != LRSC_OK) return st;
        }
        return LRSC_OK;
    }
};

DpStage::~DpStage()
{
    for(int i = 0; i < kSide; ++i) {
        if(side_done[i]) (void)hipEventDestroy(side_done[i]);
        if(side[i]) (void)hipStreamDestroy(side[i]);
    }
}

struct DpStage::Chunk {
    uint32_t begin = 0, end = 0, lds = 0;
    uint64_t jobs = 0, sbytes = 0, obytes = 0;
    DpAlignClasses classes;
    DpPipeArgs args{};
    uint32_t size() const { return end - begin; }
};

int DpStage::size_requests(std::vector<DpRequest>& reqs)
{
    for(DpRequest& r : reqs) {
        if(r.k == 0 || r.lq < r.k) return fail(LRSC_ERR_ARG, "dp request: kmer_len must satisfy 1 <= kmer_len <= query length");
        if(r.coverage > 1000) return fail(LRSC_ERR_UNSUPPORTED, "dp request: coverage above 1000 (12-bit column counters)");
        r.max_len = (uint32_t)(size_t)(r.lq * 1.1 + 20);
        r.str_cap = (std::max(r.max_len, r.k) + 3) & ~3u;
        r.ops_cap = (r.lq + r.str_cap + 1 + 3) & ~3u;
        r.cons_cap = dp_cons_capacity(r.lq);
        r.w_cols = dp_msa_columns(r.lq);
        r.cons_off = cons_total;
        cons_total += r.cons_cap;
    }
    return LRSC_OK;
}

DpStage::Chunk DpStage::plan_chunk(std::vector<DpRequest>& reqs, uint32_t begin, uint64_t budget)
{
    Chunk ch;
    ch.begin = ch.end = begin;
    while(ch.end < reqs.size()) {
        DpRequest& r = reqs[ch.end];
        r.n_str = r.cnt[0] + r.cnt[1] + r.cnt[2] + r.cnt[3];
        const uint64_t sb = (uint64_t)r.n_str * r.str_cap, ob = (uint64_t)r.n_str * r.ops_cap;
        if(ch.end > begin && ch.sbytes + ch.obytes + sb + ob + (ch.jobs + r.n_str) * (sizeof(DpJob) + sizeof(DpAlignOut)) > budget) break;
        r.job_first = ch.jobs; r.str_off = ch.sbytes; r.ops_off = ch.obytes;
        ch.jobs += r.n_str; ch.sbytes += sb; ch.obytes += ob;
        ch.classes.add(r.lq, dp_align_stage_bytes(r.lq, r.str_cap), (uint32_t)r.job_first, r.n_str);
        ch.lds = std::max(ch.lds, dp_msa_lds_bytes(r.w_cols, r.lq, r.str_cap, r.ops_cap, r.n_str));
        ++ch.end;
    }
    return ch;
}

int DpStage::run(lrsc_ctx* ctx, const Tunables& tn, const uint8_t* d_query_codes, std::vector<DpRequest>& reqs)
{
    const uint32_t n = (uint32_t)reqs.size();
    n_strings = 0; cons_total = 0;
    if(n == 0) return LRSC_OK;
    int st = size_requests(reqs);
    if(st != LRSC_OK) return st;
    HIP_TRY(d_reqs.reserve(n));
    HIP_TRY(d_msa.reserve(n));
    HIP_TRY(d_cons.reserve(cons_total));
    HIP_TRY(hipMemcpyAsync(d_reqs.p, reqs.data(), (size_t)n * sizeof(DpRequest), hipMemcpyHostToDevice, ctx->stream));
    DpPipeArgs a{};
    a.codes = d_query_codes; a.reqs = d_reqs.p; a.n_reqs = n; a.ctr = ctx->d_ctr;
    a.row_batch = tn.msa_batch;
    st = timed_launch(ctx, LRSC_K_LF, [&]() { return launch_dp_seeds(ctx->fm, a, ctx->stream); });
    if(st != LRSC_OK) return st;
    HIP_TRY(hipMemcpy(reqs.data(), d_reqs.p, (size_t)n * sizeof(DpRequest), hipMemcpyDeviceToHost));

    const uint32_t n_waves = resident_waves(ctx, 8);
    for(uint32_t begin = 0; begin < n;) {
        Chunk ch = plan_chunk(reqs, begin, tn.dp_chunk_bytes);
        if(ch.jobs >= (1ull << 32)) return fail(LRSC_ERR_UNSUPPORTED, "dp chunk: too many alignments");
        HIP_TRY(hipMemcpyAsync(d_reqs.p + begin, reqs.data() + begin, (size_t)ch.size() * sizeof(DpRequest), hipMemcpyHostToDevice, ctx->stream));
        HIP_TRY(d_strings.reserve(std::max<uint64_t>(ch.sbytes, 64)));
        HIP_TRY(d_ops.reserve(std::max<uint64_t>(ch.obytes, 64)));
        HIP_TRY(d_jobs.reserve(std::max<uint64_t>(ch.jobs, 1)));
        HIP_TRY(d_align.reserve(std::max<uint64_t>(ch.jobs, 1)));
        DpPipeArgs& c = ch.args;
        c = a;
        c.reqs = d_reqs.p + begin; c.n_reqs = ch.size(); c.n_jobs = ch.jobs;
        c.strings = d_strings.p; c.jobs = d_jobs.p; c.align = d_align.p; c.ops = d_ops.p;
        c.cons = d_cons.p; c.msa = d_msa.p + begin; c.lds_bytes = ch.lds;
        ch.classes.sort();
        st = ch.classes.upload(ctx, d_align_order, d_align_heads);
        if(st != LRSC_OK) return st;
        st = timed_launch(ctx, LRSC_K_LF, [&]() { return launch_dp_retrieve(ctx->fm, c, ctx->stream); });
        if(st == LRSC_OK) st = align_chunk(ctx, tn, reqs, ch, (uint32_t)std::min<uint64_t>(n_waves, ch.jobs));
        if(st == LRSC_OK) st = msa_chunk(ctx, tn, reqs, ch);
        if(st != LRSC_OK) return st;
        n_strings += ch.jobs;
        begin = ch.end;
    }
    return LRSC_OK;
}

int DpStage::align_chunk(lrsc_ctx* ctx, const Tunables& tn, const std::vector<DpRequest>& reqs, const Chunk& ch, uint32_t lds_waves)
{
    const uint64_t jobs = ch.jobs;
    if(jobs) {
        DpAlignArgs al{};
        al.codes = ch.args.codes; al.strings = d_strings.p; al.jobs = d_jobs.p; al.n_jobs = (uint32_t)jobs;
        al.band_width = 200; al.match_score = 1; al.gap_penalty = -1; al.mismatch_penalty = -8;
        al.ops = d_ops.p; al.out = d_align.p; al.reqs = ch.args.reqs;
        const int st = ch.classes.launch(ctx, al, lds_waves, tn.dp_align_waves, d_trace, d_seq_ws, d_align_order, d_align_heads);
        if(st != LRSC_OK) return st;
    }
    if(tn.profile && ch.begin == 0 && jobs) {
        std::vector<DpAlignOut> ao(jobs);
        (void)hipMemcpy(ao.data(), d_align.p, jobs * sizeof(DpAlignOut), hipMemcpyDeviceToHost);
        double tf = 0, tt = 0, cols = 0, na = 0, trips = 0;
        for(const DpAlignOut& o : ao) if(!o.skipped) { tf += o.t_fill; tt += o.t_trace; cols += o.total_columns; na += 1; trips += o.t_trips; }
        uint32_t big = 0;
        for(uint32_t k = 1; k <= kDpAlignClasses; ++k) if(ch.classes.cls[k].jobs > ch.classes.cls[big].jobs) big = k;
        const uint32_t nw = ch.classes.waves(big, lds_waves, tn.dp_align_waves);
        std::vector<double> wave(std::max(nw, 1u), 0.0);
        const DpOrder& order = ch.classes.order;
        for(uint32_t t = order.begin[big]; t < order.begin[big + 1]; ++t) {
            const DpAlignOut& o = ao[order.list[t]];
            wave[o.wave % wave.size()] += (double)o.t_fill + o.t_trace;
        }
        double w_max = 0, w_sum = 0;
        for(double w : wave) { w_max = std::max(w_max, w); w_sum += w; }
        std::fprintf(stderr, "[lrsc] align: %llu jobs (%.0f aligned), %.0f columns avg, per job %.0f ticks fill + %.0f ticks traceback, %.1f trips of %.2f steps; "
                             "%u waves, busiest / mean %.3f; jobs / lds B per class:",
                     (unsigned long long)jobs, na, cols / std::max(na, 1.0), tf / std::max(na, 1.0), tt / std::max(na, 1.0), trips / std::max(na, 1.0),
                     cols / std::max(trips, 1.0), (unsigned)nw, w_sum > 0 ? w_max * wave.size() / w_sum : 0.0);
        for(const DpAlignClasses::Class& k : ch.classes.cls) std::fprintf(stderr, " %llu / %u", (unsigned long long)k.jobs, k.stage_max);
        std::fprintf(stderr, " (the last from global memory)\n");
    }
    if(tn.dp_debug) {
        std::vector<DpAlignOut> ao(jobs);
        std::vector<DpJob> jj(jobs);
        (void)hipMemcpy(ao.data(), d_align.p, jobs * sizeof(DpAlignOut), hipMemcpyDeviceToHost);
        (void)hipMemcpy(jj.data(), d_jobs.p, jobs * sizeof(DpJob), hipMemcpyDeviceToHost);
        for(uint32_t i = ch.begin; i < ch.end && i < ch.begin + 3; ++i) {
            const DpRequest& r = reqs[i];
            std::fprintf(stderr, "[dp] req %u lq %u k %u cov %u cnt %u %u %u %u rows %llu %llu %llu %llu n_str %u max_len %u\n", i, r.lq, r.k,
                         r.coverage, r.cnt[0], r.cnt[1], r.cnt[2], r.cnt[3], (unsigned long long)r.row_lo[0], (unsigned long long)r.row_lo[1],
                         (unsigned long long)r.row_lo[2], (unsigned long long)r.row_lo[3], r.n_str, r.max_len);
            for(uint32_t s = 0; s < r.n_str; ++s) {
                const DpAlignOut& o = ao[r.job_first + s];
                std::fprintf(stderr, "[dp]   str %u len %u mode %u skipped %u accept %u cols %d edit %d m0 %d-%d m1 %d-%d nops %u\n", s,
                             jj[r.job_first + s].s2_len, jj[r.job_first + s].mode, o.skipped, o.accept, o.total_columns, o.edit_distance,
                             o.m0s, o.m0e, o.m1s, o.m1e, o.n_ops);
            }
        }
    }
    return LRSC_OK;
}

struct DpStage::MsaLaunch {
    DpPipeArgs args;
    size_t list_first;
    bool global_ws;
};

uint64_t DpStage::msa_buckets(const std::vector<DpRequest>& reqs, const Chunk& ch, const std::vector<uint32_t>& todo, bool force_global,
                              std::vector<MsaLaunch>& launches, std::vector<uint32_t>& lists)
{
    static const uint32_t kBuckets[] = {8u << 10, 12u << 10, 16u << 10, 20u << 10, 24u << 10, 32u << 10, 40u << 10, 80u << 10, 160u << 10, 0xFFFFFFFFu};
    uint32_t lo = 0;
    uint64_t ws_bytes = 0;
    for(uint32_t bk : kBuckets) {
        if(force_global && bk != 0xFFFFFFFFu) continue;
        const size_t first = lists.size();
        uint32_t need_max = 0;
        for(uint32_t i : todo) {
            const DpRequest& r = reqs[ch.begin + i];
            const uint32_t need = dp_msa_lds_bytes(r.w_cols, r.lq, r.str_cap, r.ops_cap, r.n_str);
            if(need > lo && need <= bk) { lists.push_back(i); need_max = std::max(need_max, need); }
        }
        lo = bk;
        if(lists.size() == first) continue;
        std::sort(lists.begin() + (std::ptrdiff_t)first, lists.end(), [&](uint32_t x, uint32_t y) {
            const DpRequest& rx = reqs[ch.begin + x]; const DpRequest& ry = reqs[ch.begin + y];
            const uint64_t wx = (uint64_t)rx.lq * rx.n_str, wy = (uint64_t)ry.lq * ry.n_str;
            return wx != wy ? wx > wy : x < y;
        });
        MsaLaunch L{ch.args, first, bk == 0xFFFFFFFFu};
        L.args.n_list = (uint32_t)(lists.size() - first);
        L.args.lds_bytes = (need_max + 15) & ~15u;
        if(L.global_ws) {
            DpPipeArgs sized = L.args;
            sized.req_list = first ? d_list.p : nullptr;
            ws_bytes = (uint64_t)L.args.lds_bytes * dp_msa_waves(sized, true);
        }
        launches.push_back(L);
    }
    return ws_bytes;
}

int DpStage::msa_chunk(lrsc_ctx* ctx, const Tunables& tn, std::vector<DpRequest>& reqs, const Chunk& ch)
{
    const uint32_t nc = ch.size(), begin = ch.begin;
    std::vector<DpMsaOut> mo(nc);
    std::vector<uint32_t> todo(nc), redo;
    for(uint32_t i = 0; i < nc; ++i) todo[i] = i;
    HIP_TRY(d_list.reserve(nc));
    while(!todo.empty()) {
        std::vector<MsaLaunch> launches;
        std::vector<uint32_t> all_lists;
        const uint64_t ws_bytes = msa_buckets(reqs, ch, todo, tn.msa_force_global, launches, all_lists);
        HIP_TRY(d_list.reserve(std::max<size_t>(all_lists.size(), 1)));
        if(ws_bytes) HIP_TRY(d_msa_ws.reserve(ws_bytes));
        HIP_TRY(hipMemcpyAsync(d_list.p, all_lists.data(), all_lists.size() * sizeof(uint32_t), hipMemcpyHostToDevice, ctx->stream));
        HIP_TRY(d_msa_ctr.reserve(std::max<size_t>(launches.size(), 16)));
        HIP_TRY(hipMemsetAsync(d_msa_ctr.p, 0, launches.size() * sizeof(uint32_t), ctx->stream));
        for(size_t j = 0; j < launches.size(); ++j) {
            MsaLaunch& L = launches[j];
            L.args.req_list = d_list.p + L.list_first;
            if(L.global_ws) L.args.msa_ws = d_msa_ws.p;
            L.args.work_ctr = d_msa_ctr.p + j;
        }
        for(int i = 0; i < kSide; ++i) {
            if(!side[i]) HIP_TRY(hipStreamCreateWithFlags(&side[i], hipStreamNonBlocking));
            if(!side_done[i]) HIP_TRY(hipEventCreateWithFlags(&side_done[i], hipEventDisableTiming));
        }
        const int st = timed_launch(ctx, LRSC_K_MSA, [&]() -> hipError_t {
            hipError_t e = hipSuccess;
            for(size_t j = 0; j < launches.size() && e == hipSuccess; ++j) {
                hipStream_t sj = side[j % kSide];
                e = hipStreamWaitEvent(sj, ctx->ev0, 0);
                if(e == hipSuccess) e = launch_dp_msa(launches[j].args, sj);
            }
            for(int i = 0; i < kSide && e == hipSuccess; ++i) {
                e = hipEventRecord(side_done[i], side[i]);
                if(e == hipSuccess) e = hipStreamWaitEvent(ctx->stream, side_done[i], 0);
            }
            return e;
        });
        if(st != LRSC_OK) return st;
        HIP_TRY(hipMemcpy(mo.data(), d_msa.p + begin, (size_t)nc * sizeof(DpMsaOut), hipMemcpyDeviceToHost));
        redo.clear();
        for(uint32_t i : todo) {
            if(mo[i].error != 1) continue;
            DpRequest& r = reqs[begin + i];
            if(r.w_cols > 64u * (r.lq + 128)) continue;
            r.w_cols *= 2;
            redo.push_back(i);
        }
        if(tn.profile && begin == 0) {
            double kt = 0, ks = 0, ki = 0, ni = 0, rows = 0, walked = 0;
            for(uint32_t i = 0; i < nc; ++i) { kt += mo[i].kc_total; ks += mo[i].kc_stage; ki += mo[i].kc_insert; ni += mo[i].n_insert; rows += mo[i].n_rows; walked += mo[i].pad; }
            std::fprintf(stderr, "[lrsc] msa: %u requests, %.1f rows avg (%.2f by the step walk), %.0f insertions avg, per request %.0f k-ticks (staging %.0f, insertions %.0f), redo %zu\n",
                         nc, rows / nc, walked / nc, ni / nc, kt / nc, ks / nc, ki / nc, redo.size());
        }
        todo = redo;
        if(!todo.empty())
            HIP_TRY(hipMemcpyAsync(d_reqs.p + begin, reqs.data() + begin, (size_t)nc * sizeof(DpRequest), hipMemcpyHostToDevice, ctx->stream));
    }
    return LRSC_OK;
}

extern "C" int lrsc_dp_align(lrsc_ctx* ctx, const char* seq, uint64_t seq_len, const lrsc_dp_job* jobs, uint32_t n, int band_width,
                             int match_score, int gap_penalty, int mismatch_penalty, lrsc_dp_result* results, char* cigar_arena,
                             uint64_t arena_cap, uint64_t* arena_used)
{
    if(!ctx || (!jobs && n) || (!results && n) || !arena_used || (!seq && seq_len)) return fail(LRSC_ERR_ARG, "null");
    *arena_used = 0;
    if(n == 0) return LRSC_OK;
    if(band_width < 2 || (band_width / 2) * 2 + 1 > (int)kDpMaxBand) return fail(LRSC_ERR_UNSUPPORTED, "band_width must be 2..254");
    if(gap_penalty > 0) return fail(LRSC_ERR_ARG, "gap_penalty must be <= 0");
    HIP_TRY(hipSetDevice(ctx->device));
    std::vector<uint8_t> codes(seq_len);
    int st = encode_acgt(seq, seq_len, codes.data());
    if(st != LRSC_OK) return st;
    std::vector<DpJob> dj(n);
    uint64_t ops_total = 0;
    DpAlignClasses classes;
    for(uint32_t i = 0; i < n; ++i) {
        const lrsc_dp_job& j = jobs[i];
        if(j.s1_off + j.s1_len > seq_len || j.s2_off + j.s2_len > seq_len) return fail(LRSC_ERR_ARG, "dp job: sequence out of range");
        if(j.s1_len > kDpMaxSeq || j.s2_len > kDpMaxSeq) return fail(LRSC_ERR_UNSUPPORTED, "dp job: sequence too long");
        DpJob& d = dj[i];
        d.s1_off = j.s1_off; d.s2_off = j.s2_off; d.s1_len = j.s1_len; d.s2_len = j.s2_len; d.start1 = j.start1; d.start2 = j.start2;
        d.mode = 0; d.req = 0; d.ops_off = ops_total;
        ops_total += (uint64_t)j.s1_len + j.s2_len + 1;
        classes.add(j.s1_len, dp_align_stage_bytes(j.s1_len, j.s2_len), i, 1);
    }
    classes.sort();
    DevBuf<uint8_t> d_codes, d_ops, d_trace, d_stage;
    DevBuf<uint32_t> d_order, d_heads;
    DevBuf<DpJob> d_jobs;
    DevBuf<DpAlignOut> d_out;
    DpAlignArgs a{};
    HIP_TRY(d_codes.reserve(std::max<uint64_t>(seq_len, 1)));
    HIP_TRY(d_ops.reserve(ops_total));
    HIP_TRY(d_jobs.reserve(n));
    HIP_TRY(d_out.reserve(n));
    HIP_TRY(hipMemcpyAsync(d_codes.p, codes.data(), seq_len, hipMemcpyHostToDevice, ctx->stream));
    HIP_TRY(hipMemcpyAsync(d_jobs.p, dj.data(), (size_t)n * sizeof(DpJob), hipMemcpyHostToDevice, ctx->stream));
    a.codes = d_codes.p; a.strings = d_codes.p; a.jobs = d_jobs.p; a.n_jobs = n; a.band_width = (uint32_t)band_width;
    a.match_score = match_score; a.gap_penalty = gap_penalty; a.mismatch_penalty = mismatch_penalty;
    a.ops = d_ops.p; a.out = d_out.p;
    st = classes.upload(ctx, d_order, d_heads);
    if(st == LRSC_OK) st = classes.launch(ctx, a, resident_waves(ctx, 2), read_tunables(ctx).dp_align_waves, d_trace, d_stage, d_order, d_heads);
    if(st != LRSC_OK) return st;
    std::vector<DpAlignOut> out(n);
    std::vector<uint8_t> ops(ops_total);
    HIP_TRY(hipMemcpy(out.data(), d_out.p, (size_t)n * sizeof(DpAlignOut), hipMemcpyDeviceToHost));
    HIP_TRY(hipMemcpy(ops.data(), d_ops.p, ops_total, hipMemcpyDeviceToHost));
    uint64_t used = 0;
    for(uint32_t i = 0; i < n; ++i) {
        const DpAlignOut& o = out[i];
        if(o.n_ops == 0xFFFFFFFFu) return fail(LRSC_ERR_DEVICE, "dp_align: traceback left the band");
        lrsc_dp_result& r = results[i];
        r.match0_start = o.m0s; r.match0_end = o.m0e; r.match1_start = o.m1s; r.match1_end = o.m1e;
        r.score = o.score; r.edit_distance = o.edit_distance; r.total_columns = o.total_columns;
        r.cigar_len = o.n_ops; r.cigar_off = used;
        if(cigar_arena && used + o.n_ops <= arena_cap)
            for(uint32_t t = 0; t < o.n_ops; ++t) cigar_arena[used + t] = (char)ops[dj[i].ops_off + o.n_ops - 1 - t];
        used += o.n_ops;
    }
    *arena_used = used;
    if(used > arena_cap || (!cigar_arena && used)) return fail(LRSC_ERR_CAPACITY, "cigar arena too small");
    return LRSC_OK;
}

extern "C" int lrsc_dp_consensus(lrsc_ctx* ctx, const char* seq, uint64_t seq_len, const lrsc_msa_query* queries, uint32_t n,
                                 lrsc_msa_result* results, char* arena, uint64_t arena_cap, uint64_t* arena_used)
{
    if(!ctx || (!queries && n) || (!results && n) || !arena_used || (!seq && seq_len)) return fail(LRSC_ERR_ARG, "null");
    *arena_used = 0;
    if(n == 0) return LRSC_OK;
    HIP_TRY(hipSetDevice(ctx->device));
    std::vector<uint8_t> codes(seq_len);
    int st = encode_acgt(seq, seq_len, codes.data());
    if(st != LRSC_OK) return st;
    std::vector<DpRequest> reqs(n);
    for(uint32_t i = 0; i < n; ++i) {
        const lrsc_msa_query& q = queries[i];
        if(q.seq_off + q.len > seq_len) return fail(LRSC_ERR_ARG, "msa query out of range");
        DpRequest& r = reqs[i];
        std::memset(&r, 0, sizeof(r));
        r.q_off = q.seq_off; r.lq = q.len; r.k = q.kmer_len; r.min_overlap = q.min_overlap; r.min_call_coverage = q.min_call_coverage;
        r.min_identity = q.min_identity; r.coverage = (uint32_t)ctx->params.pb_coverage;
    }
    DevBuf<uint8_t> d_codes;
    HIP_TRY(d_codes.reserve(std::max<uint64_t>(seq_len, 1)));
    HIP_TRY(hipMemcpyAsync(d_codes.p, codes.data(), seq_len, hipMemcpyHostToDevice, ctx->stream));
    DpStage stage;
    st = stage.run(ctx, read_tunables(ctx), d_codes.p, reqs);
    if(st != LRSC_OK) return st;
    std::vector<DpMsaOut> mo(n);
    std::vector<uint8_t> cons(stage.cons_total);
    HIP_TRY(hipMemcpy(mo.data(), stage.d_msa.p, (size_t)n * sizeof(DpMsaOut), hipMemcpyDeviceToHost));
    HIP_TRY(hipMemcpy(cons.data(), stage.d_cons.p, stage.cons_total, hipMemcpyDeviceToHost));
    uint64_t used = 0;
    for(uint32_t i = 0; i < n; ++i) {
        if(mo[i].error) return fail(LRSC_ERR_LIMIT, "msa: column capacity exceeded");
        results[i].n_rows = mo[i].n_rows; results[i].n_retrieved = reqs[i].n_str; results[i].cons_len = mo[i].cons_len; results[i].rows_by_step_walk = mo[i].pad;
        results[i].cons_off = used;
        if(arena && used + mo[i].cons_len <= arena_cap)
            for(uint32_t t = 0; t < mo[i].cons_len; ++t) arena[used + t] = "ACGT"[cons[reqs[i].cons_off + t] & 3u];
        used += mo[i].cons_len;
    }
    *arena_used = used;
    if(used > arena_cap || (!arena && used)) return fail(LRSC_ERR_CAPACITY, "consensus arena too small");
    return LRSC_OK;
}
```

longreadselfcorrect_amd/csrc/capi_internal.h:

```cpp
#pragma once
#include <hip/hip_runtime_api.h>

#include <algorithm>
#include <cstdint>
#include <cstdio>
#include <cstdlib>
#include <cstring>
#include <map>
#include <mutex>
#include <new>
#include <string>
#include <vector>

#include "../../include/lrsc.h"
#include "fm_layout.h"
#include "fm_locate.h"
#include "fm_pack.h"
#include "kernels.h"
#include "extend.h"
#include "correct_dev.h"
#include "dp_dev.h"
#include "wp.h"
#include "saipb.h"

#pragma GCC visibility push(hidden)
namespace lrsc {

int fail(int status, const std::string& msg);
int hip_fail(hipError_t e, const char* what);
#define HIP_TRY(expr)                                              \
    do {                                                           \
        hipError_t _e = (expr);                                    \
        if(_e != hipSuccess) return hip_fail(_e, #expr);           \
    } while(0)

template <class T>
struct DevBuf {
    T* p = nullptr;
    size_t cap = 0;
    ~DevBuf() { if(p) (void)hipFree(p); }
    hipError_t reserve(size_t n)
    {
        if(n <= cap) return hipSuccess;
        if(p) { (void)hipFree(p); p = nullptr; cap = 0; }
        hipError_t e = hipMalloc(reinterpret_cast<void**>(&p), n * sizeof(T));
        if(e == hipSuccess) cap = n;
        return e;
    }
};

struct DevArena {
    std::vector<DevBuf<uint8_t>*> chunks;
    size_t cur = 0, off = 0;
    ~DevArena() { for(auto* c : chunks) delete c; }
    void reset() { cur = 0; off = 0; }
    hipError_t alloc(size_t bytes, uint8_t** out)
    {
        bytes = (std::max<size_t>(bytes, 1) + 255) & ~(size_t)255;
        while(cur < chunks.size()) {
            if(chunks[cur]->cap - off >= bytes) { *out = chunks[cur]->p + off; off += bytes; return hipSuccess; }
            if(off == 0) { hipError_t e = chunks[cur]->reserve(bytes + bytes / 8); if(e != hipSuccess) return e; continue; }
            ++cur; off = 0;
        }
        auto* c = new(std::nothrow) DevBuf<uint8_t>();
        if(!c) return hipErrorOutOfMemory;
        hipError_t e = c->reserve(std::max<size_t>(bytes + bytes / 8, 64u << 20));
        if(e != hipSuccess) { delete c; return e; }
        chunks.push_back(c);
        cur = chunks.size() - 1;
        *out = c->p; off = bytes;
        return hipSuccess;
    }
};

struct Tunables {
    bool profile, wp_dump, dp_debug;
    uint32_t wp_wide_cap, wp_wave, wp_lanes;
    bool wp_begin_sort;
    uint64_t wp_prep_bytes, wp_lane_bytes;
    uint32_t wp_gen_quorum, wp_gen_wait;
    uint64_t dp_chunk_bytes;
    uint32_t dp_align_waves;
    bool msa_batch, msa_force_global;
};

struct DeviceCopy {
    void* blocks[2] = {nullptr, nullptr};
    uint64_t* dollars[2] = {nullptr, nullptr};
    uint32_t* dollar_dir[2] = {nullptr, nullptr};
    void* ktab[5] = {nullptr, nullptr, nullptr, nullptr, nullptr};
    FmIndexDev dev{};
    LocateTables locate[2];
    bool located = false;
};

struct DpStage {
    DevBuf<DpRequest> d_reqs;
    DevBuf<DpMsaOut> d_msa;
    DevBuf<uint8_t> d_cons, d_strings, d_ops, d_trace;
    DevBuf<DpJob> d_jobs;
    DevBuf<DpAlignOut> d_align;
    DevBuf<uint32_t> d_list;
    DevBuf<uint8_t> d_msa_ws, d_seq_ws;
    DevBuf<uint32_t> d_msa_ctr;
    DevBuf<uint32_t> d_align_order, d_align_heads;
    uint64_t cons_total = 0, n_strings = 0;
    static constexpr int kSide = 8;
    hipStream_t side[kSide] = {};
    hipEvent_t side_done[kSide] = {};
    ~DpStage();

    int run(lrsc_ctx* ctx, const Tunables& tn, const uint8_t* d_query_codes, std::vector<DpRequest>& reqs);

private:
    struct Chunk;
    struct MsaLaunch;
    int size_requests(std::vector<DpRequest>& reqs);
    Chunk plan_chunk(std::vector<DpRequest>& reqs, uint32_t begin, uint64_t budget);
    int align_chunk(lrsc_ctx* ctx, const Tunables& tn, const std::vector<DpRequest>& reqs, const Chunk& ch, uint32_t lds_waves);
    uint64_t msa_buckets(const std::vector<DpRequest>& reqs, const Chunk& ch, const std::vector<uint32_t>& todo, bool force_global,
                         std::vector<MsaLaunch>& launches, std::vector<uint32_t>& lists);
    int msa_chunk(lrsc_ctx* ctx, const Tunables& tn, std::vector<DpRequest>& reqs, const Chunk& ch);
};

struct CorrectScratch;

}

struct lrsc_index {
    lrsc::StrandImage image[2];
    uint64_t num_strings = 0;
    uint64_t num_symbols = 0;
    bool wide = false;
    mutable std::mutex mu;
    std::map<int, lrsc::DeviceCopy> copies;
};

struct lrsc_ctx {
    lrsc::CorrectScratch* cs = nullptr;
    const lrsc_index* index = nullptr;
    lrsc_params params{};
    int device = 0;
    hipStream_t stream = nullptr;
    hipEvent_t ev0 = nullptr, ev1 = nullptr;
    lrsc::FmIndexDev fm{};
    lrsc::DevCounters* d_ctr = nullptr;
    lrsc_kernel_stats stats[LRSC_K_COUNT]{};
    lrsc::DevBuf<uint8_t> s_in, s_codes, s_out;
    lrsc::DevBuf<uint64_t> s_off;
    lrsc::DevBuf<uint32_t> s_chunk;
    lrsc::DevBuf<int> s_flag;
    lrsc::DevBuf<uint8_t> sp_codes, sp_ws;
    lrsc::DevBuf<lrsc::SaipbSeed> sp_seeds, sp_live;
    lrsc::DevBuf<lrsc::SaipbSeedInfo> sp_info, sp_live_info;
    lrsc::DevBuf<lrsc::SaipbJob> sp_jobs;
    lrsc::DevBuf<lrsc::SaipbOut> sp_out;
    lrsc::DevBuf<char> sp_text;
    lrsc::DevBuf<uint8_t> kc_ws;
    lrsc::DevBuf<uint64_t> kc_ws_off;
    lrsc::DevBuf<lrsc_kcorrect_result> kc_res;
    lrsc::DevBuf<uint8_t> fw_ws, fw_strs, fw_best, fw_outs;
    lrsc::DevBuf<uint32_t> fw_trimmed;
    ~lrsc_ctx();
};

struct lrsc_batch {
    lrsc_ctx* ctx = nullptr;
    uint32_t n_reads = 0;
    uint64_t total_bases = 0;
    uint8_t* d_codes = nullptr;
    uint64_t* d_off = nullptr;
    uint32_t* d_chunk = nullptr;
    uint32_t n_k = 0;
    uint8_t ks[lrsc::kMaxPool]{};
    int8_t freq_index[lrsc::kMaxPool]{};
    int8_t row_of_k[64]{};
    uint32_t n_rows = 0;
    int32_t* d_freq = nullptr;
    uint8_t* d_base_counted = nullptr;
    uint8_t* d_valid = nullptr;
    bool grid_done = false;
    uint32_t min_k = 1;
    uint64_t seed_cap = 0;
    unsigned long long* d_flags = nullptr;
    uint32_t* d_zeros = nullptr;
    uint8_t* d_attr = nullptr;
    unsigned long long* d_start_bits = nullptr;
    int32_t* d_seeds = nullptr;
    uint32_t* d_seed_count = nullptr;
    float* d_thr = nullptr;
    void* d_scan_tmp = nullptr;
    size_t scan_tmp_cap = 0;
    bool seeds_done = false;
    int debug_flags = 0;
    int32_t* d_outcasts = nullptr;
    uint32_t* d_outcast_count = nullptr;
    uint8_t* d_walk_log = nullptr;
    float* d_ratio = nullptr;
    bool walk_log_done = false;
};

namespace lrsc {

Tunables read_tunables(const lrsc_ctx* ctx);
uint64_t env_bytes(const char* name, uint64_t dflt, unsigned shift);
uint32_t resident_waves(const lrsc_ctx* ctx, uint32_t per_simd);
int check_offsets(const uint64_t* off, uint32_t n_reads);
int check_walk_params(const lrsc_params& p);
void kmer_freq_table(const lrsc_params& p, double freqs[101]);
int encode_acgt(const char* seq, uint64_t n, uint8_t* codes);
int upload_and_encode(lrsc_ctx* ctx, const char* ascii, uint64_t n, uint8_t* d_codes);
int stage_reads(lrsc_ctx* ctx, const char* tool, unsigned limit_log2, const char* reads, const uint64_t* read_off, uint32_t n_reads, uint64_t slack);

void free_device_copy(DeviceCopy& dc);
int register_copy(lrsc_index* idx, int device, DeviceCopy& dc);
int image_from_device(const PackedStrand& ps, uint64_t N, uint64_t n_runs, StrandImage& im, std::string& err);
bool index_is_wide(uint64_t num_symbols);
int adopt_packed(const PackedStrand& ps, uint64_t N, uint64_t n_runs, int s, DeviceCopy& dc, StrandImage& im, std::string& err);
int adopt_packed(uint8_t* d_bwt, uint64_t N, bool wide, int s, DeviceCopy& dc, StrandImage& im, double& pack_ms, std::string& err);
int finish_index(lrsc_index* idx, int device, DeviceCopy& dc, int st, uint64_t n_dollars, int bad_status, const char* bad_msg, double ms[4],
                 int tables_slot, const char* profile_fmt);
int resident_strands(lrsc_index* idx, int device, FmStrand fs[2], bool& wide);

template <class F>
int timed_launch(lrsc_ctx* ctx, int which, F&& launch)
{
    HIP_TRY(hipMemsetAsync(ctx->d_ctr, 0, kCtrShards * sizeof(DevCounters), ctx->stream));
    HIP_TRY(hipEventRecord(ctx->ev0, ctx->stream));
    hipError_t e = launch();
    if(e != hipSuccess) return hip_fail(e, "kernel launch");
    HIP_TRY(hipEventRecord(ctx->ev1, ctx->stream));
    HIP_TRY(hipEventSynchronize(ctx->ev1));
    float ms = 0.f;
    HIP_TRY(hipEventElapsedTime(&ms, ctx->ev0, ctx->ev1));
    std::vector<DevCounters> shards(kCtrShards);
    HIP_TRY(hipMemcpy(shards.data(), ctx->d_ctr, kCtrShards * sizeof(DevCounters), hipMemcpyDeviceToHost));
    DevCounters h{};
    for(const DevCounters& d : shards) { h.rank_queries += d.rank_queries; h.block_loads += d.block_loads; h.table_loads += d.table_loads; }
    lrsc_kernel_stats& s = ctx->stats[which];
    s.launches += 1;
    s.total_ms += ms;
    s.rank_queries += h.rank_queries;
    s.block_loads += h.block_loads;
    s.table_loads += h.table_loads;
    return LRSC_OK;
}

}
#pragma GCC visibility pop
```

longreadselfcorrect_amd/csrc/dp_dev.h:

```cpp
#pragma once
#include <hip/hip_runtime_api.h>
#include <stdint.h>

#include "dp_order.h"
#include "kernels.h"

namespace lrsc {

constexpr uint32_t kDpMaxBand = 255;
constexpr uint32_t kDpTraceStride = 64;
constexpr uint32_t kDpMaxSeq = 60000;

struct DpJob {
    uint64_t s1_off, s2_off;
    uint64_t ops_off;
    uint32_t s1_len, s2_len;
    int32_t start1, start2;
    uint32_t mode;
    uint32_t req;
};

struct DpAlignOut {
    int32_t m0s, m0e, m1s, m1e;
    int32_t score, edit_distance, total_columns;
    uint32_t n_ops;
    uint32_t accept;
    uint32_t skipped;
    uint32_t t_fill, t_trace;
    uint32_t t_trips;
    uint32_t wave;
};

struct DpRequest {
    uint64_t q_off;
    uint64_t str_off, ops_off;
    uint64_t job_first;
    uint64_t cons_off;
    uint64_t row_lo[4];
    uint32_t cnt[4];
    uint32_t lq, k, max_len, str_cap, ops_cap, cons_cap, n_str;
    uint32_t w_cols;
    uint32_t min_overlap, coverage;
    int32_t min_call_coverage;
    double min_identity;
};

struct DpMsaOut {
    uint32_t n_rows;
    uint32_t cons_len;
    uint32_t error;
    uint32_t pad;
    uint32_t kc_total, kc_stage, kc_insert, n_insert;
};

struct DpPipeArgs {
    const uint8_t* codes;
    DpRequest* reqs;
    uint32_t n_reqs;
    uint64_t n_jobs;
    uint8_t* strings;
    DpJob* jobs;
    const DpAlignOut* align;
    const uint8_t* ops;
    uint8_t* cons;
    DpMsaOut* msa;
    uint32_t lds_bytes;
    const uint32_t* req_list;
    uint32_t n_list;
    uint8_t* msa_ws;
    uint32_t* work_ctr;
    uint32_t row_batch;
    DevCounters* ctr;
};

struct DpAlignArgs {
    const uint8_t* codes;
    const uint8_t* strings;
    const DpJob* jobs;
    uint32_t n_jobs;
    uint32_t band_width;
    int32_t match_score, gap_penalty, mismatch_penalty;
    uint8_t* ops;
    DpAlignOut* out;
    uint8_t* trace;
    uint64_t trace_stride;
    const DpRequest* reqs;
    const uint32_t* list;
    uint32_t n_list;
    uint32_t* head;
    uint32_t stage_max;
    uint8_t* seq_ws;
    uint64_t seq_ws_stride;
};

hipError_t launch_dp_align(const DpAlignArgs& a, uint32_t n_waves, hipStream_t stream);
hipError_t launch_dp_seeds(const FmIndexDev& fm, const DpPipeArgs& a, hipStream_t stream);
hipError_t launch_dp_retrieve(const FmIndexDev& fm, const DpPipeArgs& a, hipStream_t stream);
hipError_t launch_dp_msa(const DpPipeArgs& a, hipStream_t stream);
uint32_t dp_msa_lds_bytes(uint32_t w_cols, uint32_t lq, uint32_t str_cap, uint32_t ops_cap, uint32_t n_str);
constexpr uint32_t dp_msa_columns(uint32_t lq) { return 3 * lq + 128; }
constexpr uint32_t dp_cons_capacity(uint32_t lq) { return 2 * lq + 128; }
uint32_t dp_msa_waves(const DpPipeArgs& a, bool global);

}
```

longreadselfcorrect_amd/csrc/dp_msa.hip:

```cpp
#include <hip/hip_runtime.h>

#include "dp_dev.h"

namespace lrsc {

namespace {
constexpr uint32_t kGap = 4;
using Cnt = unsigned long long;
constexpr uint32_t kCntBits = 12;
constexpr uint32_t kMaxIns = 256;
constexpr uint32_t kUnset = 0xFEu;
__device__ __forceinline__ uint32_t cnt_get(Cnt v, uint32_t sym) { return (uint32_t)(v >> (kCntBits * sym)) & ((1u << kCntBits) - 1u); }

__device__ __forceinline__ uint32_t lane_id() { return threadIdx.x & 63u; }
__device__ __forceinline__ uint32_t mbcnt(uint64_t mask)
{
    return __builtin_amdgcn_mbcnt_hi((uint32_t)(mask >> 32), __builtin_amdgcn_mbcnt_lo((uint32_t)mask, 0u));
}
}

uint32_t dp_msa_lds_bytes(uint32_t w_cols, uint32_t lq, uint32_t str_cap, uint32_t ops_cap, uint32_t n_str)
{
    const uint32_t W = w_cols, E = n_str + 2;
    uint32_t o = 0;
    o += W * (uint32_t)sizeof(Cnt);
    o += E * 8;
    o += (lq + 2) * 4;
    o += kMaxIns * 4;
    o += kMaxIns * 2;
    o += kMaxIns;
    o += (W + 3) & ~3u;
    o += (W + 3) & ~3u;
    o += (str_cap + 7) & ~3u;
    o += (ops_cap + 3) & ~3u;
    return o;
}

template <bool GLOBAL>
__global__ __launch_bounds__(64) void dp_msa_kernel(DpPipeArgs a)
{
    extern __shared__ __attribute__((aligned(16))) uint8_t smem_lds[];
    uint8_t* smem = GLOBAL ? a.msa_ws + (uint64_t)blockIdx.x * a.lds_bytes : smem_lds;
    const uint32_t lane = lane_id();
    const uint32_t n_work = a.req_list ? a.n_list : a.n_reqs;
    for(uint32_t wi = blockIdx.x; wi < n_work;) {
        const uint32_t rq = a.req_list ? a.req_list[wi] : wi;
        uint32_t wi_next = wi + gridDim.x;
        if(a.work_ctr) {
            if(lane == 0) wi_next = gridDim.x + atomicAdd(a.work_ctr, 1u);
            wi_next = (uint32_t)__builtin_amdgcn_readfirstlane((int)wi_next);
        }
        const DpRequest R = a.reqs[rq];
        const uint64_t t_req0 = __builtin_readcyclecounter();
        uint64_t t_stage = 0, t_ins = 0;
        uint32_t n_ins = 0, n_walk = 0;
        const uint32_t W = R.w_cols, E = R.n_str + 2;
        Cnt* cnt = reinterpret_cast<Cnt*>(smem);
        uint32_t* lead = reinterpret_cast<uint32_t*>(smem + W * sizeof(Cnt));
        uint32_t* size = lead + E;
        uint32_t* bpos = size + E;
        uint32_t* insx = bpos + (R.lq + 2);
        uint16_t* insg = reinterpret_cast<uint16_t*>(insx + kMaxIns);
        uint8_t* inss = reinterpret_cast<uint8_t*>(insg + kMaxIns);
        uint8_t* T = inss + kMaxIns;
        uint8_t* Rw = T + ((W + 3) & ~3u);
        uint8_t* Sbase = Rw + ((W + 3) & ~3u);
        uint8_t* ops = Sbase + ((R.str_cap + 7) & ~3u);
        __syncthreads();
        const uint8_t* q = a.codes + R.q_off;
        for(uint32_t c = lane; c < W; c += 64) {
            Cnt z = 0;
            if(c < R.lq) { T[c] = q[c]; z = 1ull << (kCntBits * q[c]); }
            cnt[c] = z;
        }
        __syncthreads();
        uint32_t lead_b = 0, size_b = R.lq, n_el = 0, n_rows = 1;
        bool overflow = false;

        DpAlignOut A_next{};
        DpJob J_next{};
        if(R.n_str) { A_next = a.align[R.job_first]; J_next = a.jobs[R.job_first]; }
        for(uint32_t s = 0; s < R.n_str && !overflow; ++s) {
            const DpAlignOut A = A_next;
            const DpJob J = J_next;
            if(s + 1 < R.n_str) { A_next = a.align[R.job_first + s + 1]; J_next = a.jobs[R.job_first + s + 1]; }
            if(!A.accept) continue;
            ++n_rows;
            const uint64_t t_s0 = __builtin_readcyclecounter();
            __syncthreads();
            const uint32_t so = (uint32_t)(J.s2_off & 3u);
            const uint8_t* S = Sbase + so;
            {
                const uint32_t* src = reinterpret_cast<const uint32_t*>(a.strings + (J.s2_off - so));
                uint32_t* dst = reinterpret_cast<uint32_t*>(Sbase);
                for(uint32_t i = lane, n = (so + J.s2_len + 3) >> 2; i < n; i += 64) dst[i] = src[i];
                const uint32_t* osrc = reinterpret_cast<const uint32_t*>(a.ops + J.ops_off);
                uint32_t* odst = reinterpret_cast<uint32_t*>(ops);
                for(uint32_t i = lane, n = (A.n_ops + 3) >> 2; i < n; i += 64) odst[i] = osrc[i];
            }
            __syncthreads();
            const uint32_t op_last = A.n_ops - 1;
            t_stage += __builtin_readcyclecounter() - t_s0;

            uint32_t ti = 0;
            {
                uint32_t seen = 0;
                const uint32_t want = (uint32_t)A.m0s;
                for(uint32_t base = 0; base < size_b; base += 64) {
                    const uint32_t i = base + lane;
                    const bool ng = i < size_b && T[i] != kGap;
                    const uint64_t m = __ballot(ng);
                    const uint32_t nn = (uint32_t)__builtin_popcountll(m);
                    if(seen + nn > want) {
                        const uint64_t hit = __ballot(ng && mbcnt(m) == want - seen);
                        ti = base + (uint32_t)__builtin_ctzll(hit);
                        break;
                    }
                    seen += nn;
                }
            }
            const uint32_t tl = lead_b;
            const uint32_t il = ti + tl;
            bool batched = false;
            if(a.row_batch && A.n_ops > 0 && !(ti == 0 && ops[op_last] == 'I')) {
                const uint32_t ti0 = ti, m1s = (uint32_t)A.m1s;
                uint32_t nbr = 0;
                for(uint32_t base = ti0; base < size_b; base += 64) {
                    const uint32_t i = base + lane;
                    const bool in = i < size_b;
                    const bool ng = in && T[i] != kGap;
                    const uint64_t m = __ballot(ng);
                    if(ng) { const uint32_t b = nbr + mbcnt(m); if(b < R.lq + 1) bpos[b] = i; }
                    if(in) Rw[i] = ng ? (uint8_t)kUnset : (uint8_t)kGap;
                    nbr += (uint32_t)__builtin_popcountll(m);
                }
                bool bad = nbr > R.lq + 1;
                if(lane == 0 && !bad) bpos[nbr] = size_b;
                __syncthreads();
                uint32_t md_tot = 0, mi_tot = 0, st_tot = 0, run_carry = 0, last_y = 0;
                for(uint32_t cb = 0; cb < A.n_ops && !bad; cb += 64) {
                    const uint32_t j = cb + lane;
                    const bool valid = j < A.n_ops;
                    const uint32_t op = valid ? (uint32_t)ops[op_last - j] : 0u;
                    const bool isM = op == 'M', isD = op == 'D', isI = op == 'I';
                    const uint64_t mMD = __ballot(isM || isD), mMI = __ballot(isM || isI);
                    const uint32_t brel = md_tot + mbcnt(mMD);
                    const uint32_t inc = m1s + mi_tot + mbcnt(mMI);
                    const uint64_t lower = mMD & ((1ull << lane) - 1ull);
                    const uint32_t run_start = lower ? cb + 64u - (uint32_t)__builtin_clzll(lower) : run_carry;
                    const uint32_t i_rank = j - run_start;
                    bool lane_bad = valid && !(isM || isD || isI);
                    uint32_t y = 0, G = 0;
                    bool st = false, fill = false;
                    if((isM || isD) && brel >= nbr) lane_bad = true;
                    if(isI && brel >= nbr) lane_bad = true;
                    if(!lane_bad && valid) {
                        const uint32_t pb = bpos[brel];
                        if(isI) {
                            if(brel > 0) { const uint32_t pp = bpos[brel - 1]; G = pb - pp - 1; y = pp + 1 + i_rank; }
                            fill = i_rank < G; st = !fill;
                            if(st) y = pb - 1;
                        } else y = pb;
                    }
                    const uint64_t mS = __ballot(st);
                    const uint32_t k = st_tot + mbcnt(mS);
                    if(st && k >= kMaxIns) lane_bad = true;
                    if(__ballot(lane_bad)) { bad = true; break; }
                    const uint32_t sym = (isM || isI) ? (inc < J.s2_len ? (uint32_t)S[inc] : 0u) : kGap;
                    if(isM || isD || fill) Rw[y] = (uint8_t)sym;
                    if(st) { insx[k] = y + 1; inss[k] = (uint8_t)sym; }
                    md_tot += (uint32_t)__builtin_popcountll(mMD);
                    mi_tot += (uint32_t)__builtin_popcountll(mMI);
                    st_tot += (uint32_t)__builtin_popcountll(mS);
                    if(mMD) run_carry = cb + 64u - (uint32_t)__builtin_clzll(mMD);
                    if(cb + 64 >= A.n_ops) last_y = (uint32_t)__shfl((int)y, (int)((A.n_ops - 1) & 63u));
                }
                __syncthreads();
                if(!bad) {
                    batched = true;
                    const uint32_t nin = st_tot;
                    if(nin) {
                        const uint64_t t_i0 = __builtin_readcyclecounter();
                        n_ins += nin;
                        if(size_b + nin > W || lead_b + size_b + nin > W) { overflow = true; break; }
                        for(uint32_t k0 = 0; k0 < nin; k0 += 64) {
                            const uint32_t k = k0 + lane;
                            const uint32_t xg = k < nin ? insx[k] + tl : 0u;
                            uint32_t g = 0;
                            for(uint32_t e = 0; e < n_el; ++e) { const uint32_t le = lead[e], se = size[e]; g += (le < xg && xg - le < se) ? 1u : 0u; }
                            if(k < nin) insg[k] = (uint16_t)g;
                        }
                        __syncthreads();
                        for(uint32_t e0 = 0; e0 < n_el; e0 += 64) {
                            const uint32_t e = e0 + lane;
                            if(e < n_el) {
                                const uint32_t le = lead[e], se = size[e];
                                uint32_t before = 0, inside = 0;
                                for(uint32_t k = 0; k < nin; ++k) {
                                    const uint32_t xg = insx[k] + tl;
                                    before += xg <= le ? 1u : 0u;
                                    inside += (le < xg && xg - le < se) ? 1u : 0u;
                                }
                                lead[e] = le + before; size[e] = se + inside;
                            }
                        }
                        const uint32_t x0 = insx[0];
                        for(uint32_t hi = size_b; hi > x0;) {
                            const uint32_t n = hi - x0 < 64 ? hi - x0 : 64;
                            const uint32_t yy = hi - 1 - lane;
                            Cnt v = 0; uint8_t t = 0, r = 0; uint32_t sh = 0;
                            if(lane < n) {
                                v = cnt[yy + tl]; t = T[yy]; r = Rw[yy];
                                uint32_t lo = 0, hi2 = nin;
                                while(lo < hi2) { const uint32_t mid = (lo + hi2) >> 1; if(insx[mid] <= yy) lo = mid + 1; else hi2 = mid; }
                                sh = lo;
                            }
                            __syncthreads();
                            if(lane < n && sh) { cnt[yy + sh + tl] = v; T[yy + sh] = t; Rw[yy + sh] = r; }
                            __syncthreads();
                            hi -= n;
                        }
                        for(uint32_t k0 = 0; k0 < nin; k0 += 64) {
                            const uint32_t k = k0 + lane;
                            if(k < nin) {
                                const uint32_t np = insx[k] + k;
                                T[np] = (uint8_t)kGap; Rw[np] = inss[k];
                                cnt[np + tl] = (Cnt)((uint32_t)insg[k] + 1u) << (kCntBits * kGap);
                            }
                        }
                        size_b += nin;
                        __syncthreads();
                        t_ins += __builtin_readcyclecounter() - t_i0;
                    }
                    const uint32_t nout = last_y + 1 - ti0 + nin;
                    if(nout > W) { overflow = true; break; }
                    for(uint32_t z0 = 0; z0 < nout; z0 += 64) {
                        const uint32_t z = z0 + lane;
                        if(z < nout) {
                            const uint32_t sym = Rw[ti0 + z];
                            if(sym <= kGap && ti0 + z + tl < W) cnt[ti0 + z + tl] += 1ull << (kCntBits * sym);
                        }
                    }
                    __syncthreads();
                    if(n_el >= E) { overflow = true; break; }
                    if(lane == 0) { lead[n_el] = il; size[n_el] = nout; }
                    ++n_el;
                    __syncthreads();
                }
            }
            if(batched) continue;
            ++n_walk;
            uint32_t inc = (uint32_t)A.m1s, cig = 0, nout = 0;
            uint32_t tb = 0xFFFFFF00u, ob = 0xFFFFFF00u, sb = 0xFFFFFF00u, Tw = 0, Ow = 0, Sw = 0, acc = 0;
            auto getT = [&](uint32_t i) -> uint32_t {
                if(i - tb >= 64u) { tb = i; const uint32_t j = i + lane; Tw = j < size_b ? (uint32_t)T[j] : 0xFFu; }
                return (uint32_t)__builtin_amdgcn_readlane((int)Tw, (int)(i - tb));
            };
            auto getO = [&](uint32_t i) -> uint32_t {
                if(i - ob >= 64u) { ob = i; const uint32_t j = i + lane; Ow = j < A.n_ops ? (uint32_t)ops[op_last - j] : 0u; }
                return (uint32_t)__builtin_amdgcn_readlane((int)Ow, (int)(i - ob));
            };
            auto getS = [&](uint32_t i) -> uint32_t {
                if(i - sb >= 64u) { sb = i; const uint32_t j = i + lane; Sw = j < J.s2_len ? (uint32_t)S[j] : 0u; }
                return (uint32_t)__builtin_amdgcn_readlane((int)Sw, (int)(i - sb));
            };
            auto flush = [&](uint32_t first, uint32_t n) {
                const uint32_t col = il + first + lane;
                if(lane < n && col < W) cnt[col] += 1ull << (kCntBits * acc);
            };
            while(cig < A.n_ops) {
                ti = (uint32_t)__builtin_amdgcn_readfirstlane((int)ti);
                cig = (uint32_t)__builtin_amdgcn_readfirstlane((int)cig);
                inc = (uint32_t)__builtin_amdgcn_readfirstlane((int)inc);
                const uint32_t tsym = getT(ti);
                const uint32_t op = getO(cig);
                uint32_t sym;
                if(tsym == kGap) {
                    if(op == 'I') { sym = getS(inc); ++inc; ++cig; }
                    else sym = kGap;
                } else if(op == 'M') { sym = getS(inc); ++inc; ++cig; }
                else if(op == 'D') { sym = kGap; ++cig; }
                else {
                    const uint64_t t_i0 = __builtin_readcyclecounter();
                    ++n_ins;
                    const uint32_t c = ti + tl;
                    uint32_t ngap = 0;
                    for(uint32_t e0 = 0; e0 < n_el; e0 += 64) {
                        const uint32_t e = e0 + lane;
                        bool inside = false;
                        if(e < n_el) {
                            const uint32_t le = lead[e], se = size[e];
                            if(c <= le) lead[e] = le + 1;
                            else if(c - le < se) { size[e] = se + 1; inside = true; }
                        }
                        ngap += (uint32_t)__builtin_popcountll(__ballot(inside));
                    }
                    const uint32_t end_b = lead_b + size_b;
                    bool base_inside = false;
                    if(c <= lead_b) lead_b += 1;
                    else if(c - lead_b < size_b) {
                        base_inside = true;
                        const uint32_t ip = c - lead_b;
                        if(size_b + 1 > W) { overflow = true; break; }
                        for(uint32_t hi = size_b; hi > ip;) {
                            const uint32_t n = hi - ip < 64 ? hi - ip : 64;
                            const uint32_t i = hi - 1 - lane;
                            uint8_t v = 0;
                            if(lane < n) v = T[i];
                            __syncthreads();
                            if(lane < n) T[i + 1] = v;
                            __syncthreads();
                            hi -= n;
                        }
                        if(lane == 0) T[ip] = (uint8_t)kGap;
                        size_b += 1;
                        tb = 0xFFFFFF00u;
                    }
                    if(c < end_b) {
                        if(end_b + 1 > W) { overflow = true; break; }
                        for(uint32_t hi = end_b; hi > c;) {
                            const uint32_t n = hi - c < 64 ? hi - c : 64;
                            const uint32_t i = hi - 1 - lane;
                            Cnt v = 0;
                            if(lane < n) v = cnt[i];
                            __syncthreads();
                            if(lane < n) cnt[i + 1] = v;
                            __syncthreads();
                            hi -= n;
                        }
                    }
                    if(c < W && lane == 0) cnt[c] = (Cnt)(ngap + (base_inside ? 1u : 0u)) << (kCntBits * kGap);
                    __syncthreads();
                    t_ins += __builtin_readcyclecounter() - t_i0;
                    sym = getS(inc); ++inc; ++cig;
                }
                if(nout >= W) { overflow = true; break; }
                acc = lane == (nout & 63u) ? sym : acc;
                ++nout;
                if((nout & 63u) == 0) flush(nout - 64, 64);
                ++ti;
            }
            if(overflow) break;
            if((nout & 63u) != 0) flush(nout & ~63u, nout & 63u);
            __syncthreads();
            if(n_el >= E) { overflow = true; break; }
            if(lane == 0) { lead[n_el] = il; size[n_el] = nout; }
            ++n_el;
            __syncthreads();
        }

        uint32_t cons_len = 0;
        uint8_t* cons = a.cons + R.cons_off;
        if(!overflow) {
            for(uint32_t base = 0; base < size_b; base += 64) {
                const uint32_t i = base + lane;
                uint32_t sym = kGap;
                if(i < size_b && lead_b + i < W) {
                    const Cnt v = cnt[lead_b + i];
                    int max_count = -1; uint32_t max_symbol = 0;
#pragma unroll
                    for(uint32_t x = 0; x < 5; ++x)
                        if((int)cnt_get(v, x) > max_count) { max_count = (int)cnt_get(v, x); max_symbol = x; }
                    const uint32_t base_symbol = T[i];
                    const int base_count = (int)cnt_get(v, base_symbol);
                    sym = (max_count >= base_count && base_count < R.min_call_coverage) ? max_symbol : base_symbol;
                }
                const bool keep = i < size_b && sym != kGap;
                const uint64_t m = __ballot(keep);
                if(keep) {
                    const uint32_t pos = cons_len + mbcnt(m);
                    if(pos < R.cons_cap) cons[pos] = (uint8_t)sym;
                }
                cons_len += (uint32_t)__builtin_popcountll(m);
            }
            if(cons_len > R.cons_cap) { overflow = true; cons_len = 0xFFFFFFFFu; }
        }
        if(lane == 0) {
            DpMsaOut o;
            o.n_rows = n_rows; o.cons_len = overflow ? 0 : cons_len; o.error = !overflow ? 0u : cons_len == 0xFFFFFFFFu ? 2u : 1u; o.pad = n_walk;
            o.kc_total = (uint32_t)((__builtin_readcyclecounter() - t_req0) >> 10); o.kc_stage = (uint32_t)(t_stage >> 10);
            o.kc_insert = (uint32_t)(t_ins >> 10); o.n_insert = n_ins;
            a.msa[rq] = o;
        }
        wi = wi_next;
    }
}

uint32_t dp_msa_waves(const DpPipeArgs& a, bool global)
{
    int cus = 256, dev = 0;
    (void)hipGetDevice(&dev);
    (void)hipDeviceGetAttribute(&cus, hipDeviceAttributeMultiprocessorCount, dev);
    uint32_t per_cu = global ? 8u : (a.lds_bytes ? (160u * 1024u) / a.lds_bytes : 16u);
    per_cu = per_cu < 1 ? 1 : per_cu > 32 ? 32 : per_cu;
    uint32_t n_waves = (uint32_t)cus * per_cu;
    const uint32_t n_work = a.req_list ? a.n_list : a.n_reqs;
    return n_waves > n_work ? n_work : n_waves;
}

hipError_t launch_dp_msa(const DpPipeArgs& a, hipStream_t stream)
{
    const uint32_t n_work = a.req_list ? a.n_list : a.n_reqs;
    if(n_work == 0) return hipSuccess;
    if(a.msa_ws) {
        hipLaunchKernelGGL(dp_msa_kernel<true>, dim3(dp_msa_waves(a, true)), dim3(64), 0, stream, a);
        return hipGetLastError();
    }
    if(a.lds_bytes > 160 * 1024) return hipErrorInvalidValue;
    if(a.lds_bytes > 64 * 1024) {
        const hipError_t e = hipFuncSetAttribute(reinterpret_cast<const void*>(dp_msa_kernel<false>),
                                                 hipFuncAttributeMaxDynamicSharedMemorySize, (int)a.lds_bytes);
        if(e != hipSuccess) return e;
    }
    hipLaunchKernelGGL(dp_msa_kernel<false>, dim3(dp_msa_waves(a, false)), dim3(64), a.lds_bytes, stream, a);
    return hipGetLastError();
}

}
```

longreadselfcorrect_amd/csrc/wp.h:

```cpp
#pragma once
#include <hip/hip_runtime_api.h>
#include <stdint.h>

#include "correct_dev.h"
#include "dp_dev.h"
#include "extend.h"

namespace lrsc {

enum : uint32_t { kWpFmValid = 1u, kWpDpValid = 2u, kWpGeomBad = 4u };
enum : uint32_t { kWpReqFm = 0u, kWpReqDp = 1u };

struct alignas(16) WpSlot {
    uint32_t read, it;
    uint64_t src_lo, src_hi;
    uint8_t k, next, rtou, flags;
    uint8_t dp_k, max_front, pad1, pad2;
    uint64_t dp_src_lo, dp_src_hi;
    uint32_t lq, gap, trg_len, pathw;
    uint32_t dp_lq;
    int32_t dp_total_freq;
    uint8_t* q;
    uint8_t* dpq;
    uint8_t* prep;
    uint32_t* path;
    int32_t code;
    uint32_t path_len, match_i, steps;
    uint32_t dp_rows, dp_cons_len, dp_error, leaf_steps;
    const uint8_t* dp_cons;
};

struct alignas(16) WpStatic {
    uint64_t root[4];
    uint64_t tmask0, tmask1;
    uint32_t n9f, n9r;
    uint32_t pad[2];
};

struct WpPrepLayout { uint32_t item9f, item9r, term, next9f, next9r, head9, head5, next5, flags5, total; };
__host__ __device__ inline WpPrepLayout wp_prep_layout(uint32_t lq, uint32_t trg_len, uint32_t seed_size, uint32_t min_overlap, uint32_t psz)
{
    const uint32_t n9 = lq >= seed_size ? lq - seed_size + 1 : 0, n5 = lq >= 5 ? lq - 4 : 0;
    const uint32_t nT = trg_len >= min_overlap ? trg_len - min_overlap + 1 : 0;
    WpPrepLayout L;
    uint32_t o = (uint32_t)sizeof(WpStatic);
    L.item9f = o; o += n9 * 16u;
    L.item9r = o; o += n9 * 16u;
    L.term = o;   o = (o + nT * 4u * psz + 15u) & ~15u;
    L.next9f = o; o += n9 * 2u;
    L.next9r = o; o += n9 * 2u;
    L.head9 = (o + 1u) & ~1u; o = L.head9 + 1024u;
    L.head5 = o;  o += 2048u;
    L.next5 = o;  o += n5 * 2u;
    L.flags5 = o; o += n5;
    L.total = (o + 63u) & ~63u;
    return L;
}

struct WpLaneLayout { uint32_t leaves, rings, results, paths, total; };
__host__ __device__ inline WpLaneLayout wp_lane_layout(uint32_t lbytes, uint32_t pathw)
{
    WpLaneLayout L;
    uint32_t o = 0;
    L.leaves = o;  o = (o + (32u + kMaxChildren) * lbytes + 15u) & ~15u;
    L.rings = o;   o += 32u * 100u * 8u;
    L.results = o; o += kMaxResults * (uint32_t)sizeof(WalkResultRec);
    L.paths = o;   o += (32u + kMaxResults) * pathw * 4u;
    L.total = (o + 63u) & ~63u;
    return L;
}

struct WpWideLayout { uint32_t leaves, rings, results, paths, total; };
__host__ __device__ inline WpWideLayout wp_wide_layout(uint32_t lbytes, uint32_t pathw, uint32_t cap)
{
    WpWideLayout L;
    uint32_t o = 0;
    L.leaves = o;  o = (o + 5u * cap * lbytes + 15u) & ~15u;
    L.rings = o;   o += cap * 100u * 8u;
    L.results = o; o += wide_results(cap) * (uint32_t)sizeof(WalkResultRec);
    L.paths = o;   o += (cap + wide_results(cap)) * pathw * 4u;
    L.total = (o + 63u) & ~63u;
    return L;
}

struct WpReadWork {
    uint64_t out_off;
    uint64_t piece_off;
    uint64_t slot_first;
    uint32_t out_cap, piece_cap;
    uint32_t n_seeds;
    uint32_t pad;
};

struct WpRead {
    int64_t c[10];
    uint64_t steps;
    uint32_t n_pieces, out_len, merge;
    int32_t error;
    uint32_t state;
    uint32_t it;
    int32_t next, first_type;
    int32_t s_seed_len, s_end, s_end_best, s_max_fixed, s_is_repeat;
    uint32_t started;
};

struct WpDpItem {
    uint64_t q;
    uint32_t slot, lq, k;
    int32_t total_freq;
};

struct WpRequest { uint32_t slot, kind; };

struct WpArgs {
    const uint8_t* codes;
    const uint64_t* read_off;
    const int32_t* seeds;
    const uint32_t* seed_count;
    uint32_t n_reads, min_k;
    uint32_t r0, r1;
    uint64_t slot_base;
    const WpReadWork* work;
    WpRead* reads;
    WpSlot* slots;
    uint64_t n_slots;
    uint32_t seed_size, min_overlap, max_leaves;
    int32_t start_kmer_len, next_target, split, no_dp;
    uint64_t pb_coverage;
    double pacbio_error_rate;
    const double* freqs_of_kmer_size;
    uint32_t psz, lbytes;
    const uint32_t* list;
    const WpRequest* reqs;
    uint32_t n_list;
    uint64_t *sz_q, *sz_prep, *sz_path;
    uint8_t *arena_q, *arena_prep, *arena_path;
    uint32_t* plan_stats;
    uint32_t* sort_key;
    uint32_t* queue;
    uint8_t* lane_ws;
    uint32_t lane_ws_bytes, lane_pathw, n_lanes;
    uint32_t lane_stride;
    uint32_t general_quorum_pct, general_max_wait;
    uint32_t auto_dp;
    WpDpItem* dp_items;
    uint32_t* n_dp_items;
    uint32_t dp_items_cap;
    const DpRequest* dp_reqs;
    const DpMsaOut* dp_msa;
    const uint8_t* dp_cons;
    uint32_t n_dp;
    uint8_t* out_codes;
    uint32_t* piece_start;
    WpRequest* req_out;
    uint32_t* n_req_out;
    uint32_t req_cap;
    uint8_t* walk_log;
    DevCounters* ctr;
    unsigned long long* prof;
    uint32_t escalate;
    uint32_t* sort9;
    uint32_t* n_sort9;
    uint32_t begin_sort;
    unsigned long long* begin_stats;
};

constexpr uint32_t kWpPathwSmall = 64, kWpPathwMid = 256;

enum WpSmall : uint32_t {
    kWpSmallPlanStats = 0,
    kWpSmallQueue = 4,
    kWpSmallDpItems = 5,
    kWpSmallReqOut = 6,
    kWpSmallSort9 = 7,
    kWpSmallExtQueue = 8,
    kWpSmallSideQueue = 9,
    kWpSmallSideDpItems = 12,
    kWpSmallWideQueue = 13,
    kWpSmallWideCount = 14,
    kWpSmallWords = 16
};

hipError_t launch_wp_bounds(const WpArgs& a, ReadPlan* plan, hipStream_t stream);
hipError_t launch_wp_plan(const WpArgs& a, hipStream_t stream);
hipError_t launch_wp_materialize(const WpArgs& a, hipStream_t stream);
hipError_t launch_wp_prepare(const FmIndexDev& fm, const WpArgs& a, hipStream_t stream);
hipError_t launch_wp_begin(const FmIndexDev& fm, const WpArgs& a, hipStream_t stream);
hipError_t launch_wp_extend(const FmIndexDev& fm, const WpArgs& a, hipStream_t stream);
hipError_t launch_wp_extend_wave(const FmIndexDev& fm, const WpArgs& a, hipStream_t stream);
hipError_t launch_wp_wide_collect(const WpArgs& a, uint32_t* out, uint32_t* n_out, hipStream_t stream);
hipError_t launch_wp_extend_wide(const FmIndexDev& fm, const WpArgs& a, hipStream_t stream);
hipError_t launch_wp_dp_collect(const WpArgs& a, const WpDpItem* items, hipStream_t stream);
hipError_t launch_wp_stitch(const WpArgs& a, hipStream_t stream);
hipError_t launch_wp_gather(const WpArgs& a, const uint64_t* dst_off, char* dst, hipStream_t stream);
hipError_t wp_scan(uint64_t* v, uint64_t n, void** tmp, size_t* tmp_cap, hipStream_t stream);
hipError_t wp_sort_list(const uint32_t* keys, uint32_t* keys_tmp, uint32_t* list, uint32_t* list_tmp, uint32_t n, void** tmp, size_t* tmp_cap, hipStream_t stream);

}
```

longreadselfcorrect_amd/csrc/wp_wave.hip:

```cpp
#define LRSC_WALK_FN __device__ __forceinline__
#define LRSC_WALK_NOINLINE
#include <hip/hip_runtime.h>

#include "walk_device.h"
#include "wp.h"
#include "wp_walk.h"

namespace lrsc {

#ifndef LRSC_WP_EXTEND_OCC
#define LRSC_WP_EXTEND_OCC 2
#endif

namespace {

__device__ __forceinline__ uint32_t wave_or(uint32_t v)
{
    for(int o = 32; o > 0; o >>= 1) v |= (uint32_t)__shfl_xor((int)v, o, 64);
    return first_u32(v);
}
__device__ __forceinline__ uint32_t kth_bit(uint32_t m, uint32_t k)
{
    for(uint32_t j = 0; j < k; ++j) m &= m - 1u;
    return m ? (uint32_t)__builtin_ctz(m) : 0u;
}

template <bool WIDE>
__device__ __forceinline__ uint64_t wave_select(Walk<WIDE>& W, uint64_t LowerBound, uint64_t UpperBound, const Leaf<typename Lay<WIDE>::pos_t>* leaves,
                                                uint32_t n, uint32_t lane)
{
    using P = typename Lay<WIDE>::pos_t;
    const uint32_t U = (uint32_t)UpperBound, Lw = (uint32_t)LowerBound;
    const bool h0 = lane < n, h1 = lane + 64 < n;
    uint64_t s0lo = 0, s0hi = 0, s1lo = 0, s1hi = 0;
    if(h0) { s0lo = leaves[lane].suf_lo; s0hi = leaves[lane].suf_hi; }
    if(h1) { s1lo = leaves[lane + 64].suf_lo; s1hi = leaves[lane + 64].suf_hi; }
    IvT<P> f0{}, r0{}, f1{}, r1{};
    int mx = 0;
    if(h0) { W.select_first(s0lo, s0hi, U, Lw, f0, r0); const int fr = (int)(isize(f0.lo, f0.hi) + isize(r0.lo, r0.hi)); mx = fr > mx ? fr : mx; }
    if(h1) { W.select_first(s1lo, s1hi, U, Lw, f1, r1); const int fr = (int)(isize(f1.lo, f1.hi) + isize(r1.lo, r1.hi)); mx = fr > mx ? fr : mx; }
    mx = wave_max(mx);
    if(mx - (int)W.freqsOfKmerSize[LowerBound] < 5) return LowerBound;
    for(uint64_t i = 1; i <= UpperBound - LowerBound; i++) {
        const uint32_t t = (uint32_t)(UpperBound - LowerBound - i);
        mx = 0;
        if(h0) { W.select_next(s0lo, s0hi, U, t, f0, r0); const int fr = (int)(isize(f0.lo, f0.hi) + isize(r0.lo, r0.hi)); mx = fr > mx ? fr : mx; }
        if(h1) { W.select_next(s1lo, s1hi, U, t, f1, r1); const int fr = (int)(isize(f1.lo, f1.hi) + isize(r1.lo, r1.hi)); mx = fr > mx ? fr : mx; }
        mx = wave_max(mx);
        if(mx - (int)W.freqsOfKmerSize[LowerBound + i] < 5) return LowerBound + i;
    }
    return UpperBound;
}

template <bool WIDE>
__device__ __forceinline__ void wave_attempt(Walk<WIDE>& W, uint32_t lane)
{
    using P = typename Lay<WIDE>::pos_t;
    const uint32_t n = W.n_cur;
    const bool have = lane < n;
    Leaf<P> par = {};
    if(have) par = W.cur[lane];
    const double minimumErrorRate = wave_min(have && par.localErr < 1.0 ? par.localErr : 1.0);
    bool keep = false;
    if(have) {
        const double errorRateDiff = par.localErr - minimumErrorRate;
        keep = !((errorRateDiff > 0.05 && W.currentLength > W.localK / 2) || (errorRateDiff > 0.1 && W.currentLength > 15));
    }
    W.ring_free |= wave_or(have && !keep ? 1u << par.ring : 0u);
    W.path_free |= wave_or(have && !keep ? 1u << par.path : 0u);
    const uint64_t below = lanes_below(lane);
    const uint64_t km = __ballot(keep);
    const uint32_t pos = popc64(km & below);
    const uint32_t n_kept = popc64(km);
    if(keep && pos != lane) W.cur[pos] = par;
    W.n_cur = n_kept;

    const uint32_t nr0 = W.n_rank, nb0 = W.n_blk;
    typename Walk<WIDE>::Ext ext[4];
    uint32_t mask = 0;
    if(keep) {
        int count = 0;
        while(count < 2) {
            if(count == 1 && !(par.localErr == minimumErrorRate && n_kept > 1)) break;
            uint64_t tc;
            mask = W.getFMIndexExtensions_v(par.flo, par.fhi, par.rlo, par.rhi, par.tailLetterCount, par.suf_lo, ext, tc);
            if(mask != 0) break;
            W.min_SA_threshold--;
            count++;
        }
        W.min_SA_threshold += (uint64_t)count;
    }
    uint32_t off = 0, total = 0;
#pragma unroll
    for(uint32_t b = 0; b < 4; ++b) {
        const uint64_t m = __ballot(((mask >> b) & 1u) != 0);
        off += popc64(m & below);
        total += popc64(m);
    }
    if(off > kMaxChildren) { W.n_rank = nr0; W.n_blk = nb0; }
    if(total > kMaxChildren) { W.error = LRSC_WALK_ERR_CHILDREN; return; }
    const int highfreqThreshold = W.PBcoverage > 60 ? (int)((uint64_t)(W.PBcoverage / 60) * 3) : 3;
    uint32_t hf = 0, k = off;
#pragma unroll
    for(uint32_t b = 0; b < 4; ++b) {
        if(!((mask >> b) & 1u)) continue;
        const Leaf<P> ch = W.make_child(par, pos, b, ext[b]);
        if(ch.kmerFrequency > highfreqThreshold) ++hf;
        W.nxt[k++] = ch;
    }
    W.n_highfreq = wave_sum(hf);
    W.n_nxt = total;
    wave_sync();
}

template <bool WIDE>
__device__ __forceinline__ void wave_extend(Walk<WIDE>& W, uint32_t lane)
{
    W.n_nxt = 0;
    uint64_t t = W.tick();
    if(W.currentKmerSize > W.maxOverlap) { wave_refine(W, W.cur, W.n_cur, W.maxOverlap, lane); wave_sync(); }
    W.tock(1, t);
    t = W.tick();
    wave_attempt(W, lane);
    W.tock(2, t);
    if(W.error) return;
    if(W.n_nxt == 0) {
        const uint64_t LowerBound = (W.currentKmerSize - 2) > W.minOverlap ? (W.currentKmerSize - 2) : W.minOverlap;
        const uint64_t ReduceSize = wave_select(W, LowerBound, W.currentKmerSize, W.cur, W.n_cur, lane);
        wave_refine(W, W.cur, W.n_cur, ReduceSize, lane);
        wave_sync();
        wave_attempt(W, lane);
        if(W.error) return;
        if(W.n_nxt == 0) {
            W.min_SA_threshold--;
            wave_attempt(W, lane);
            W.min_SA_threshold++;
            if(W.error) return;
        }
    }
    if(W.n_nxt != 0) {
        W.currentLength++;
        W.currentKmerSize++;
        if(W.isInsufficientFreqs(W.n_highfreq, W.n_nxt)) {
            const uint64_t LowerBound = (W.currentKmerSize - 2) > W.minOverlap ? (W.currentKmerSize - 2) : W.minOverlap;
            const uint64_t ReduceSize = wave_select(W, LowerBound, W.currentKmerSize, W.nxt, W.n_nxt, lane);
            wave_refine(W, W.nxt, W.n_nxt, ReduceSize, lane);
        }
    }
}

template <bool WIDE>
__device__ __forceinline__ void wave_prune(Walk<WIDE>& W, uint32_t lane, Leaf<typename Lay<WIDE>::pos_t>& c0, Leaf<typename Lay<WIDE>::pos_t>& c1)
{
    const uint64_t currSeedIdx = W.currentLength - W.seedSize;
    const uint64_t indelOffset = W.seedSize + W.maxIndelSize;
    const uint64_t smallSeedIdx = currSeedIdx <= indelOffset ? 0 : currSeedIdx - indelOffset;
    const uint64_t largeSeedIdx = (currSeedIdx + indelOffset) >= (W.Lq - W.seedSize) ? (W.Lq - W.seedSize) : currSeedIdx + indelOffset;
    const uint32_t n = W.n_nxt;
    bool a0 = false, a1 = false;
    uint32_t hc = 0;
    if(lane < n) {
        c0 = W.nxt[lane];
        W.template prune_leaf<true>(c0, W.rings + (uint64_t)c0.ring * 100, currSeedIdx, smallSeedIdx, largeSeedIdx);
        W.nxt[lane] = c0;
        a0 = c0.alive != 0;
        if(a0) hc |= 1u << c0.parent;
    }
    if(lane + 64 < n) {
        c1 = W.nxt[lane + 64];
        W.template prune_leaf<true>(c1, W.rings + (uint64_t)c1.ring * 100, currSeedIdx, smallSeedIdx, largeSeedIdx);
        W.nxt[lane + 64] = c1;
        a1 = c1.alive != 0;
        if(a1) hc |= 1u << c1.parent;
    }
    W.alive_lo = __ballot(a0);
    W.alive_hi = __ballot(a1);
    W.has_child = wave_or(hc);
}

template <bool WIDE>
__device__ __forceinline__ void wave_commit(Walk<WIDE>& W, uint32_t lane, Leaf<typename Lay<WIDE>::pos_t>& c0, Leaf<typename Lay<WIDE>::pos_t>& c1)
{
    using P = typename Lay<WIDE>::pos_t;
    uint64_t t = W.tick();
    const uint64_t am0 = W.alive_lo, am1 = W.alive_hi;
    const uint32_t survivors = popc64(am0) + popc64(am1);
    ++W.steps;
    if(survivors > W.maxLeaves) {
        wave_sync();
        if(lane == 0 && W.currentLength >= W.minLength)
            for(uint32_t c = 0; c < W.n_nxt; ++c) {
                if((((c < 64 ? am0 >> c : am1 >> (c - 64)) & 1ull)) == 0) continue;
                const Leaf<P>& par = W.cur[W.nxt[c].parent];
                W.terminated_leaf(W.nxt[c], W.paths + (uint64_t)par.path * W.pathw, par.path_len, (int)W.nxt[c].ext);
                if(W.error) break;
            }
        W.n_results = first_u32(W.n_results);
        W.error = (int)first_u32((uint32_t)W.error);
        W.n_cur = survivors;
        W.ended = true;
        return;
    }
    const uint64_t below = lanes_below(lane);
    uint32_t fr = 0, fp = 0;
    if(lane < W.n_cur && !((W.has_child >> lane) & 1u)) { fr = 1u << W.cur[lane].ring; fp = 1u << W.cur[lane].path; }
    W.ring_free |= wave_or(fr);
    W.path_free |= wave_or(fp);
    const bool a0 = ((am0 >> lane) & 1ull) != 0, a1 = ((am1 >> lane) & 1ull) != 0;
    const uint32_t p0 = c0.parent, p1 = c1.parent;
    const uint64_t m0 = am0 & below, m1 = am1 & below;
    const uint32_t prev0 = (uint32_t)__shfl((int)p0, m0 ? 63 - __builtin_clzll(m0) : (int)lane, 64);
    const uint32_t prev1 = (uint32_t)__shfl((int)p1, m1 ? 63 - __builtin_clzll(m1) : (int)lane, 64);
    const uint32_t last0 = am0 ? lane_u32(p0, 63u - (uint32_t)__builtin_clzll(am0)) : 0xFFFFFFFFu;
    const bool fur0 = a0 && m0 != 0 && prev0 == p0;
    const bool fur1 = a1 && (m1 != 0 ? prev1 == p1 : last0 == p1);
    const uint64_t f0 = __ballot(fur0), f1 = __ballot(fur1);
    const uint32_t n_further = popc64(f0) + popc64(f1);
    uint32_t r0 = c0.ring, q0 = c0.path, r1 = c1.ring, q1 = c1.path;
    if(fur0) { const uint32_t k = popc64(f0 & below); r0 = kth_bit(W.ring_free, k); q0 = kth_bit(W.path_free, k); }
    if(fur1) { const uint32_t k = popc64(f0) + popc64(f1 & below); r1 = kth_bit(W.ring_free, k); q1 = kth_bit(W.path_free, k); }
    for(uint32_t j = 0; j < n_further; ++j) { W.ring_free &= W.ring_free - 1u; W.path_free &= W.path_free - 1u; }
    wave_copy_slots(W, f0, c0, r0, q0, lane);
    wave_copy_slots(W, f1, c1, r1, q1, lane);
    if(a0 && !fur0) {
        W.rings[(uint64_t)c0.ring * 100 + (c0.hist_size - 1) % 100] = c0.globalErr;
        path_set(W.paths + (uint64_t)c0.path * W.pathw, c0.path_len, c0.ext);
    }
    if(a1 && !fur1) {
        W.rings[(uint64_t)c1.ring * 100 + (c1.hist_size - 1) % 100] = c1.globalErr;
        path_set(W.paths + (uint64_t)c1.path * W.pathw, c1.path_len, c1.ext);
    }
    c0.ring = (uint16_t)r0; c0.path = (uint16_t)q0; c0.path_len++;
    c1.ring = (uint16_t)r1; c1.path = (uint16_t)q1; c1.path_len++;
    W.tock(5, t);
    t = W.tick();
    int hit0 = -1, hit1 = -1;
    uint64_t h0 = 0, h1 = 0;
    if(W.currentLength >= W.minLength) {
        if(a0) hit0 = W.term_scan(c0);
        if(a1) hit1 = W.term_scan(c1);
        const bool need0 = hit0 >= 0 && c0.res_first == -1, need1 = hit1 >= 0 && c1.res_first == -1;
        const uint64_t n0 = __ballot(need0), n1 = __ballot(need1);
        bool bad = false;
        if(need0) { const uint32_t k = W.n_results + popc64(n0 & below); if(k >= kMaxResults) bad = true; else c0.res_first = (int)k + 1; }
        if(need1) { const uint32_t k = W.n_results + popc64(n0) + popc64(n1 & below); if(k >= kMaxResults) bad = true; else c1.res_first = (int)k + 1; }
        if(hit0 >= 0) c0.res_second = hit0;
        if(hit1 >= 0) c1.res_second = hit1;
        if(__ballot(bad)) W.error = LRSC_WALK_ERR_RESULTS;
        W.n_results += popc64(n0) + popc64(n1);
        h0 = __ballot(hit0 >= 0);
        h1 = __ballot(hit1 >= 0);
    }
    const bool swap = 4u * survivors <= (W.cur == W.leaf_small ? 32u : kMaxChildren);
    Leaf<P>* dest = swap ? W.nxt : W.cur;
    if(a0) dest[popc64(m0)] = c0;
    if(a1) dest[popc64(am0) + popc64(m1)] = c1;
    if(swap) { Leaf<P>* t2 = W.cur; W.cur = W.nxt; W.nxt = t2; }
    W.n_cur = survivors;
    wave_sync();
    if(!W.error && (h0 | h1)) {
        wave_store_results(W, h0, c0, hit0, lane);
        wave_store_results(W, h1, c1, hit1, lane);
        wave_sync();
    }
    W.tock(6, t);
}

template <bool WIDE>
__device__ __forceinline__ bool wave_step(Walk<WIDE>& W, uint32_t lane)
{
    using P = typename Lay<WIDE>::pos_t;
    if(W.ended || W.error || !(W.n_cur != 0 && W.n_cur <= W.maxLeaves && W.currentLength <= W.maxLength)) return false;
    W.leaf_steps += W.n_cur;
    if(W.n_cur > W.max_front) W.max_front = W.n_cur;
    wave_sync();
    uint64_t t = W.tick();
    wave_extend(W, lane);
    W.tock(0, t);
    if(W.error) return true;
    t = W.tick();
    Leaf<P> c0 = {}, c1 = {};
    wave_prune(W, lane, c0, c1);
    W.tock(4, t);
    wave_commit(W, lane, c0, c1);
    return true;
}

}

template <bool WIDE>
__global__ __launch_bounds__(64, LRSC_WP_EXTEND_OCC) void wp_extend_wave_kernel(FmIndexDev fm, WpArgs a)
{
    using P = typename Lay<WIDE>::pos_t;
    __shared__ __attribute__((aligned(16))) uint32_t mtab[MaskTabSize<WIDE>::value];
    init_mask_table<WIDE>(mtab);
    const uint32_t lane = threadIdx.x;
    const uint32_t wave = blockIdx.x;
    Walk<WIDE> W;
    wp_walk_consts(W, fm, a, mtab);
    const WpLaneLayout LL = wp_lane_layout(a.lbytes, a.lane_pathw);
    uint8_t* lws = a.lane_ws + (uint64_t)(wave < a.n_lanes ? wave : 0u) * a.lane_ws_bytes;
    Leaf<P>* const leaf_base = reinterpret_cast<Leaf<P>*>(lws + LL.leaves);
    W.rings = reinterpret_cast<double*>(lws + LL.rings);
    W.results = reinterpret_cast<WalkResultRec*>(lws + LL.results);
    W.paths = reinterpret_cast<uint32_t*>(lws + LL.paths);
    W.pathw = a.lane_pathw;
    W.rpaths = W.paths + (uint64_t)32 * a.lane_pathw;

    Leaf<P> L;
    uint32_t pw = 0;
    uint64_t pr[8] = {0, 0, 0, 0, 0, 0, 0, 0};
    uint64_t t_refill = 0, t_finish = 0, n_fast = 0;
    const bool prof = a.prof != nullptr;
    if(prof) W.prof = pr;
    const uint64_t t_loop0 = prof ? __builtin_readcyclecounter() : 0;
    if(wave < a.n_lanes)
    while(true) {
        const uint64_t tr0 = prof ? __builtin_readcyclecounter() : 0;
        uint32_t i = 0;
        if(lane == 0) i = atomicAdd(a.queue, 1u);
        i = first_u32(i);
        if(i >= a.n_list) break;
        if(a.reqs && a.reqs[i].kind != kWpReqFm) continue;
        const uint32_t si = a.list ? a.list[i] : (uint32_t)a.slot_base + i;
        if(a.slots[si].flags & kWpGeomBad) continue;
        W.cur = leaf_base; W.nxt = leaf_base + 32; W.leaf_small = leaf_base;
        wp_walk_bind(W, a, a.slots[si]);
        const uint64_t steps0 = W.steps;
        if(prof) t_refill += __builtin_readcyclecounter() - tr0;
        while(true) {
            int r = 2;
            if(W.can_fast()) r = wave_fast_steps(W, L, pw, lane, prof, pr[7], n_fast);
            if(r == 2) r = wave_step(W, lane) ? 1 : 0;
            if(r == 0) break;
        }
        const uint64_t tf0 = prof ? __builtin_readcyclecounter() : 0;
        wave_sync();
        if(lane == 0) wp_walk_finish(W, a, si, steps0);
        if(prof) t_finish += __builtin_readcyclecounter() - tf0;
    }
    if(prof && wave < a.n_lanes && lane == 0) {
        for(int j = 0; j < 8; ++j) atomicAdd(&a.prof[j], (unsigned long long)pr[j]);
        atomicAdd(&a.prof[8], (unsigned long long)t_refill);
        atomicAdd(&a.prof[9], (unsigned long long)t_finish);
        atomicAdd(&a.prof[10], (unsigned long long)(__builtin_readcyclecounter() - t_loop0));
        atomicAdd(&a.prof[11], (unsigned long long)W.steps);
        atomicAdd(&a.prof[12], (unsigned long long)n_fast);
    }
    flush_counters(a.ctr, W.n_rank, W.n_blk);
}

hipError_t launch_wp_extend_wave(const FmIndexDev& fm, const WpArgs& a, hipStream_t stream)
{
    if(a.n_list == 0 || a.n_lanes == 0) return hipSuccess;
    if(fm.wide) hipLaunchKernelGGL(wp_extend_wave_kernel<true>, dim3(a.n_lanes), dim3(64), 0, stream, fm, a);
    else        hipLaunchKernelGGL(wp_extend_wave_kernel<false>, dim3(a.n_lanes), dim3(64), 0, stream, fm, a);
    return hipGetLastError();
}

}
```

Baseline: 146.9.

## Co-schedule MSA with side walks: LDS-aware buckets, balanced stream deal, stream copies

Sizes the MSA LDS buckets and wave counts from the LDS left over after the concurrently resident side extend-wave kernels, instead of fixed sizes based on 160 KiB. MSA launches are now dealt to 3 side streams by greedy work balancing rather than round-robin over 8. The side walk stream gets the lowest priority. Blocking hipMemcpy calls become stream-ordered async copies plus a stream sync, and DevBuf reserve over-allocates by 25% to cut realloc churn. Together these aim to let DP MSA overlap better with side walking and to reduce host synchronization and allocation overhead, at the cost of smaller LDS budgets per MSA workgroup.

```diff
diff --git a/longreadselfcorrect_amd/csrc/capi_batch.cpp b/longreadselfcorrect_amd/csrc/capi_batch.cpp
--- a/longreadselfcorrect_amd/csrc/capi_batch.cpp
+++ b/longreadselfcorrect_amd/csrc/capi_batch.cpp
@@ -164,7 +164,7 @@
     HIP_TRY(hipMalloc(reinterpret_cast<void**>(&b->d_thr), 3 * 52 * sizeof(float)));
     float thr[3 * 52];
     (void)lrsc_kmer_thresholds(ctx->params.pb_coverage, thr);
-    HIP_TRY(hipMemcpy(b->d_thr, thr, sizeof(thr), hipMemcpyHostToDevice));
+    COPY_TRY(ctx, b->d_thr, thr, sizeof(thr), hipMemcpyHostToDevice);
     return LRSC_OK;
 }
 
diff --git a/longreadselfcorrect_amd/csrc/capi_core.cpp b/longreadselfcorrect_amd/csrc/capi_core.cpp
--- a/longreadselfcorrect_amd/csrc/capi_core.cpp
+++ b/longreadselfcorrect_amd/csrc/capi_core.cpp
@@ -103,6 +103,7 @@
     t.dp_chunk_bytes = env_bytes("LRSC_DP_CHUNK_MB", 16ull << 30, 20);
     t.dp_align_waves = env_clamped("LRSC_DP_ALIGN_WAVES", 0, 0, kIntMax);
     t.msa_force_global = std::getenv("LRSC_MSA_FORCE_GLOBAL") != nullptr;
+    t.msa_lds_max = env_clamped("LRSC_MSA_LDS_MAX", 0, 1, kIntMax);
     { const char* e = std::getenv("LRSC_MSA_BATCH"); t.msa_batch = !(e && e[0] == '0'); }
     t.profile = std::getenv("LRSC_CORRECT_PROFILE") != nullptr;
     t.wp_dump = std::getenv("LRSC_WP_DUMP") != nullptr;
diff --git a/longreadselfcorrect_amd/csrc/capi_correct.cpp b/longreadselfcorrect_amd/csrc/capi_correct.cpp
--- a/longreadselfcorrect_amd/csrc/capi_correct.cpp
+++ b/longreadselfcorrect_amd/csrc/capi_correct.cpp
@@ -208,7 +208,11 @@
         a.prof = sc.d_prof.p;
         a.begin_stats = sc.d_prof.p + 32;
     }
-    if(!sc.side) HIP_TRY(hipStreamCreateWithFlags(&sc.side, hipStreamNonBlocking));
+    if(!sc.side) {
+        int least = 0, greatest = 0;
+        HIP_TRY(hipDeviceGetStreamPriorityRange(&least, &greatest));
+        HIP_TRY(hipStreamCreateWithPriority(&sc.side, hipStreamNonBlocking, least));
+    }
     if(!sc.ev_ready) HIP_TRY(hipEventCreateWithFlags(&sc.ev_ready, hipEventDisableTiming));
     return LRSC_OK;
 }
@@ -266,12 +270,11 @@
     a.list = nullptr; a.reqs = nullptr;
     if(R.index != 0) {
         uint32_t n_req = 0;
-        HIP_TRY(hipStreamSynchronize(ctx->stream));
-        HIP_TRY(hipMemcpy(&n_req, a.n_req_out, sizeof(uint32_t), hipMemcpyDeviceToHost));
+        COPY_TRY(ctx, &n_req, a.n_req_out, sizeof(uint32_t), hipMemcpyDeviceToHost);
         if(n_req == 0) { *done = true; return LRSC_OK; }
         if(n_req > n) return fail(LRSC_ERR_LIMIT, "walk-parallel flow: request list overflow");
         hreq.resize(n_req);
-        HIP_TRY(hipMemcpy(hreq.data(), sc.d_req.p, (size_t)n_req * sizeof(WpRequest), hipMemcpyDeviceToHost));
+        COPY_TRY(ctx, hreq.data(), sc.d_req.p, (size_t)n_req * sizeof(WpRequest), hipMemcpyDeviceToHost);
         std::sort(hreq.begin(), hreq.end(), [](const WpRequest& x, const WpRequest& y) { return x.slot < y.slot; });
         hlist.resize(n_req);
         for(uint32_t i = 0; i < n_req; ++i) hlist[i] = hreq[i].slot;
@@ -346,7 +349,7 @@
     if(tn.wp_wave == 2) stride = 64;
     const WpLaneLayout LL = wp_lane_layout(lbytes, pathw);
     const uint64_t slots = tn.wp_lanes / 64;
-    const uint64_t share = side ? std::max<uint64_t>(1, slots / 2) : slots;
+    const uint64_t share = side ? wp_side_waves(tn) : slots;
     uint64_t lanes = std::min<uint64_t>(stride == 1 ? (((uint64_t)count + 63) & ~63ull) : count, share * 64 / stride);
     lanes = std::max<uint64_t>(1, std::min<uint64_t>(lanes, (tn.wp_lane_bytes / (side ? 4 : 1)) / LL.total));
     if(stride == 1) lanes = std::max<uint64_t>(64, lanes & ~63ull);
@@ -427,11 +430,11 @@
 int WpFlow::fetch_items(DevBuf<WpDpItem>& d_list, const uint32_t* d_count, uint32_t cap, Round& R, std::vector<WpDpItem>& out)
 {
     uint32_t cnt = 0;
-    HIP_TRY(hipMemcpy(&cnt, d_count, sizeof(uint32_t), hipMemcpyDeviceToHost));
+    COPY_TRY(ctx, &cnt, d_count, sizeof(uint32_t), hipMemcpyDeviceToHost);
     if(cnt > cap) return fail(LRSC_ERR_LIMIT, "walk-parallel flow: DP item list overflow");
     R.n_items += cnt;
     out.resize(cnt);
-    if(cnt) HIP_TRY(hipMemcpy(out.data(), d_list.p, (size_t)cnt * sizeof(WpDpItem), hipMemcpyDeviceToHost));
+    if(cnt) COPY_TRY(ctx, out.data(), d_list.p, (size_t)cnt * sizeof(WpDpItem), hipMemcpyDeviceToHost);
     std::sort(out.begin(), out.end(), [](const WpDpItem& x, const WpDpItem& y) { return x.slot < y.slot; });
     return LRSC_OK;
 }
@@ -483,7 +486,7 @@
     lrsc_kernel_stats& s = ctx->stats[LRSC_K_EXTEND];
     s.total_ms += ms;
     std::vector<DevCounters> shards(kCtrShards);
-    HIP_TRY(hipMemcpy(shards.data(), sc.d_ctr2.p, kCtrShards * sizeof(DevCounters), hipMemcpyDeviceToHost));
+    COPY_TRY(ctx, shards.data(), sc.d_ctr2.p, kCtrShards * sizeof(DevCounters), hipMemcpyDeviceToHost);
     for(const DevCounters& dcn : shards) {
         s.rank_queries += dcn.rank_queries;
         s.block_loads += dcn.block_loads;
@@ -575,10 +578,9 @@
                            uint64_t* n_pieces_out, uint64_t* out_used)
 {
     std::vector<WpRead> ro(n);
-    HIP_TRY(hipStreamSynchronize(ctx->stream));
-    HIP_TRY(hipMemcpy(ro.data(), sc.d_reads.p, (size_t)n * sizeof(WpRead), hipMemcpyDeviceToHost));
+    COPY_TRY(ctx, ro.data(), sc.d_reads.p, (size_t)n * sizeof(WpRead), hipMemcpyDeviceToHost);
     std::vector<uint32_t> pieces(std::max<uint64_t>(piece_total, 1));
-    if(piece_total) HIP_TRY(hipMemcpy(pieces.data(), sc.d_pieces.p, (size_t)piece_total * sizeof(uint32_t), hipMemcpyDeviceToHost));
+    if(piece_total) COPY_TRY(ctx, pieces.data(), sc.d_pieces.p, (size_t)piece_total * sizeof(uint32_t), hipMemcpyDeviceToHost);
     std::vector<uint64_t> dst_off(n + 1, 0);
     uint64_t n_pieces = 0;
     for(uint32_t r = 0; r < n; ++r) {
diff --git a/longreadselfcorrect_amd/csrc/capi_dp.cpp b/longreadselfcorrect_amd/csrc/capi_dp.cpp
--- a/longreadselfcorrect_amd/csrc/capi_dp.cpp
+++ b/longreadselfcorrect_amd/csrc/capi_dp.cpp
@@ -1,4 +1,5 @@
 #include "capi_internal.h"
+#include "dp_deal.h"
 
 using namespace lrsc;
 
@@ -114,13 +115,29 @@
     return ch;
 }
 
+int DpStage::msa_lds_budget(lrsc_ctx* ctx, const Tunables& tn, uint32_t* budget) const
+{
+    uint32_t wg_lds = 0;
+    HIP_TRY(wp_extend_wave_static_lds(ctx->fm.wide != 0, &wg_lds));
+    int cus = 256;
+    HIP_TRY(hipDeviceGetAttribute(&cus, hipDeviceAttributeMultiprocessorCount, ctx->device));
+    const uint64_t wgs_per_cu = (wp_side_waves(tn) + (uint64_t)cus - 1) / (uint64_t)cus;
+    const uint64_t held = wgs_per_cu * (((uint64_t)wg_lds + kLdsGranule - 1) / kLdsGranule * kLdsGranule);
+    uint32_t b = held < kLdsPerCu ? (uint32_t)(kLdsPerCu - held) : 0u;
+    if(tn.msa_lds_max) b = std::min(b, tn.msa_lds_max);
+    *budget = b;
+    return LRSC_OK;
+}
+
 int DpStage::run(lrsc_ctx* ctx, const Tunables& tn, const uint8_t* d_query_codes, std::vector<DpRequest>& reqs)
 {
     const uint32_t n = (uint32_t)reqs.size();
     n_strings = 0; cons_total = 0;
     if(n == 0) return LRSC_OK;
     int st = size_requests(reqs);
-    if(st != LRSC_OK) return st;
+    if(st == LRSC_OK) st = msa_lds_budget(ctx, tn, &lds_budget);
+    if(st != LRSC_OK) return st;
+    if(tn.profile) std::fprintf(stderr, "[lrsc] msa: LDS budget per CU %u B\n", (unsigned)lds_budget);
     HIP_TRY(d_reqs.reserve(n));
     HIP_TRY(d_msa.reserve(n));
     HIP_TRY(d_cons.reserve(cons_total));
@@ -130,7 +147,7 @@
     a.row_batch = tn.msa_batch;
     st = timed_launch(ctx, LRSC_K_LF, [&]() { return launch_dp_seeds(ctx->fm, a, ctx->stream); });
     if(st != LRSC_OK) return st;
-    HIP_TRY(hipMemcpy(reqs.data(), d_reqs.p, (size_t)n * sizeof(DpRequest), hipMemcpyDeviceToHost));
+    COPY_TRY(ctx, reqs.data(), d_reqs.p, (size_t)n * sizeof(DpRequest), hipMemcpyDeviceToHost);
 
     const uint32_t n_waves = resident_waves(ctx, 8);
     for(uint32_t begin = 0; begin < n;) {
@@ -218,15 +235,20 @@
     DpPipeArgs args;
     size_t list_first;
     bool global_ws;
+    uint64_t work;
 };
 
 uint64_t DpStage::msa_buckets(const std::vector<DpRequest>& reqs, const Chunk& ch, const std::vector<uint32_t>& todo, bool force_global,
-                              std::vector<MsaLaunch>& launches, std::vector<uint32_t>& lists)
-{
-    static const uint32_t kBuckets[] = {8u << 10, 12u << 10, 16u << 10, 20u << 10, 24u << 10, 32u << 10, 40u << 10, 80u << 10, 160u << 10, 0xFFFFFFFFu};
+                              std::vector<MsaLaunch>& launches, std::vector<uint32_t>& lists) const
+{
+    static const uint32_t kWgsPerCu[] = {20, 13, 10, 8, 6, 5, 4, 2, 1};
+    uint32_t buckets[sizeof(kWgsPerCu) / sizeof(kWgsPerCu[0]) + 1];
+    uint32_t nb = 0;
+    for(uint32_t w : kWgsPerCu) buckets[nb++] = (lds_budget / w) & ~15u;
+    buckets[nb++] = 0xFFFFFFFFu;
     uint32_t lo = 0;
     uint64_t ws_bytes = 0;
-    for(uint32_t bk : kBuckets) {
+    for(uint32_t bk : buckets) {
         if(force_global && bk != 0xFFFFFFFFu) continue;
         const size_t first = lists.size();
         uint32_t need_max = 0;
@@ -242,13 +264,14 @@
             const uint64_t wx = (uint64_t)rx.lq * rx.n_str, wy = (uint64_t)ry.lq * ry.n_str;
             return wx != wy ? wx > wy : x < y;
         });
-        MsaLaunch L{ch.args, first, bk == 0xFFFFFFFFu};
+        MsaLaunch L{ch.args, first, bk == 0xFFFFFFFFu, 0};
+        for(size_t t = first; t < lists.size(); ++t) { const DpRequest& r = reqs[ch.begin + lists[t]]; L.work += (uint64_t)r.lq * r.n_str; }
         L.args.n_list = (uint32_t)(lists.size() - first);
         L.args.lds_bytes = (need_max + 15) & ~15u;
         if(L.global_ws) {
             DpPipeArgs sized = L.args;
             sized.req_list = first ? d_list.p : nullptr;
-            ws_bytes = (uint64_t)L.args.lds_bytes * dp_msa_waves(sized, true);
+            ws_bytes = (uint64_t)L.args.lds_bytes * dp_msa_waves(sized, true, lds_budget);
         }
         launches.push_back(L);
     }
@@ -281,21 +304,23 @@
             if(!side[i]) HIP_TRY(hipStreamCreateWithFlags(&side[i], hipStreamNonBlocking));
             if(!side_done[i]) HIP_TRY(hipEventCreateWithFlags(&side_done[i], hipEventDisableTiming));
         }
+        std::vector<DpDealLaunch> dl;
+        for(const MsaLaunch& L : launches) dl.push_back({L.work, L.global_ws ? 0u : L.args.lds_bytes});
+        const std::vector<std::vector<uint32_t>> deal = dp_deal(dl, (uint32_t)kSide);
         const int st = timed_launch(ctx, LRSC_K_MSA, [&]() -> hipError_t {
             hipError_t e = hipSuccess;
-            for(size_t j = 0; j < launches.size() && e == hipSuccess; ++j) {
-                hipStream_t sj = side[j % kSide];
-                e = hipStreamWaitEvent(sj, ctx->ev0, 0);
-                if(e == hipSuccess) e = launch_dp_msa(launches[j].args, sj);
+            for(size_t i = 0; i < deal.size() && e == hipSuccess; ++i) {
+                if(deal[i].empty()) continue;
+                e = hipStreamWaitEvent(side[i], ctx->ev0, 0);
+                for(size_t t = 0; t < deal[i].size() && e == hipSuccess; ++t) e = launch_dp_msa(launches[deal[i][t]].args, lds_budget, side[i]);
+                if(e == hipSuccess) e = hipEventRecord(side_done[i], side[i]);
             }
-            for(int i = 0; i < kSide && e == hipSuccess; ++i) {
-                e = hipEventRecord(side_done[i], side[i]);
-                if(e == hipSuccess) e = hipStreamWaitEvent(ctx->stream, side_done[i], 0);
-            }
+            for(size_t i = 0; i < deal.size() && e == hipSuccess; ++i)
+                if(!deal[i].empty()) e = hipStreamWaitEvent(ctx->stream, side_done[i], 0);
             return e;
         });
         if(st != LRSC_OK) return st;
-        HIP_TRY(hipMemcpy(mo.data(), d_msa.p + begin, (size_t)nc * sizeof(DpMsaOut), hipMemcpyDeviceToHost));
+        COPY_TRY(ctx, mo.data(), d_msa.p + begin, (size_t)nc * sizeof(DpMsaOut), hipMemcpyDeviceToHost);
         redo.clear();
         for(uint32_t i : todo) {
             if(mo[i].error != 1) continue;
@@ -363,8 +388,8 @@
     if(st != LRSC_OK) return st;
     std::vector<DpAlignOut> out(n);
     std::vector<uint8_t> ops(ops_total);
-    HIP_TRY(hipMemcpy(out.data(), d_out.p, (size_t)n * sizeof(DpAlignOut), hipMemcpyDeviceToHost));
-    HIP_TRY(hipMemcpy(ops.data(), d_ops.p, ops_total, hipMemcpyDeviceToHost));
+    COPY_TRY(ctx, out.data(), d_out.p, (size_t)n * sizeof(DpAlignOut), hipMemcpyDeviceToHost);
+    COPY_TRY(ctx, ops.data(), d_ops.p, ops_total, hipMemcpyDeviceToHost);
     uint64_t used = 0;
     for(uint32_t i = 0; i < n; ++i) {
         const DpAlignOut& o = out[i];
@@ -409,8 +434,8 @@
     if(st != LRSC_OK) return st;
     std::vector<DpMsaOut> mo(n);
     std::vector<uint8_t> cons(stage.cons_total);
-    HIP_TRY(hipMemcpy(mo.data(), stage.d_msa.p, (size_t)n * sizeof(DpMsaOut), hipMemcpyDeviceToHost));
-    HIP_TRY(hipMemcpy(cons.data(), stage.d_cons.p, stage.cons_total, hipMemcpyDeviceToHost));
+    COPY_TRY(ctx, mo.data(), stage.d_msa.p, (size_t)n * sizeof(DpMsaOut), hipMemcpyDeviceToHost);
+    COPY_TRY(ctx, cons.data(), stage.d_cons.p, stage.cons_total, hipMemcpyDeviceToHost);
     uint64_t used = 0;
     for(uint32_t i = 0; i < n; ++i) {
         if(mo[i].error) return fail(LRSC_ERR_LIMIT, "msa: column capacity exceeded");
diff --git a/longreadselfcorrect_amd/csrc/capi_internal.h b/longreadselfcorrect_amd/csrc/capi_internal.h
--- a/longreadselfcorrect_amd/csrc/capi_internal.h
+++ b/longreadselfcorrect_amd/csrc/capi_internal.h
@@ -42,9 +42,15 @@
     hipError_t reserve(size_t n)
     {
         if(n <= cap) return hipSuccess;
+        size_t want = cap ? std::max(n, cap + cap / 4) : n;
         if(p) { (void)hipFree(p); p = nullptr; cap = 0; }
-        hipError_t e = hipMalloc(reinterpret_cast<void**>(&p), n * sizeof(T));
-        if(e == hipSuccess) cap = n;
+        hipError_t e = hipMalloc(reinterpret_cast<void**>(&p), want * sizeof(T));
+        if(e != hipSuccess && want > n) {
+            (void)hipGetLastError();
+            p = nullptr; want = n;
+            e = hipMalloc(reinterpret_cast<void**>(&p), want * sizeof(T));
+        }
+        if(e == hipSuccess) cap = want; else p = nullptr;
         return e;
     }
 };
@@ -82,6 +88,7 @@
     uint64_t dp_chunk_bytes;
     uint32_t dp_align_waves;
     bool msa_batch, msa_force_global;
+    uint32_t msa_lds_max;
 };
 
 struct DeviceCopy {
@@ -105,7 +112,8 @@
     DevBuf<uint32_t> d_msa_ctr;
     DevBuf<uint32_t> d_align_order, d_align_heads;
     uint64_t cons_total = 0, n_strings = 0;
-    static constexpr int kSide = 8;
+    uint32_t lds_budget = 0;
+    static constexpr int kSide = 3;
     hipStream_t side[kSide] = {};
     hipEvent_t side_done[kSide] = {};
     ~DpStage();
@@ -117,9 +125,10 @@
     struct MsaLaunch;
     int size_requests(std::vector<DpRequest>& reqs);
     Chunk plan_chunk(std::vector<DpRequest>& reqs, uint32_t begin, uint64_t budget);
+    int msa_lds_budget(lrsc_ctx* ctx, const Tunables& tn, uint32_t* budget) const;
     int align_chunk(lrsc_ctx* ctx, const Tunables& tn, const std::vector<DpRequest>& reqs, const Chunk& ch, uint32_t lds_waves);
     uint64_t msa_buckets(const std::vector<DpRequest>& reqs, const Chunk& ch, const std::vector<uint32_t>& todo, bool force_global,
-                         std::vector<MsaLaunch>& launches, std::vector<uint32_t>& lists);
+                         std::vector<MsaLaunch>& launches, std::vector<uint32_t>& lists) const;
     int msa_chunk(lrsc_ctx* ctx, const Tunables& tn, std::vector<DpRequest>& reqs, const Chunk& ch);
 };
 
@@ -205,6 +214,7 @@
 Tunables read_tunables(const lrsc_ctx* ctx);
 uint64_t env_bytes(const char* name, uint64_t dflt, unsigned shift);
 uint32_t resident_waves(const lrsc_ctx* ctx, uint32_t per_simd);
+inline uint64_t wp_side_waves(const Tunables& tn) { return std::max<uint64_t>(1, tn.wp_lanes / 64 / 2); }
 int check_offsets(const uint64_t* off, uint32_t n_reads);
 int check_walk_params(const lrsc_params& p);
 void kmer_freq_table(const lrsc_params& p, double freqs[101]);
@@ -221,6 +231,18 @@
 int finish_index(lrsc_index* idx, int device, DeviceCopy& dc, int st, uint64_t n_dollars, int bad_status, const char* bad_msg, double ms[4],
                  int tables_slot, const char* profile_fmt);
 int resident_strands(lrsc_index* idx, int device, FmStrand fs[2], bool& wide);
+
+inline int copy_sync(lrsc_ctx* ctx, void* dst, const void* src, size_t bytes, hipMemcpyKind kind)
+{
+    if(bytes) HIP_TRY(hipMemcpyAsync(dst, src, bytes, kind, ctx->stream));
+    HIP_TRY(hipStreamSynchronize(ctx->stream));
+    return LRSC_OK;
+}
+#define COPY_TRY(ctx, dst, src, bytes, kind)                                   \
+    do {                                                                       \
+        const int _st = lrsc::copy_sync((ctx), (dst), (src), (bytes), (kind)); \
+        if(_st != LRSC_OK) return _st;                                         \
+    } while(0)
 
 template <class F>
 int timed_launch(lrsc_ctx* ctx, int which, F&& launch)
@@ -234,7 +256,7 @@
     float ms = 0.f;
     HIP_TRY(hipEventElapsedTime(&ms, ctx->ev0, ctx->ev1));
     std::vector<DevCounters> shards(kCtrShards);
-    HIP_TRY(hipMemcpy(shards.data(), ctx->d_ctr, kCtrShards * sizeof(DevCounters), hipMemcpyDeviceToHost));
+    COPY_TRY(ctx, shards.data(), ctx->d_ctr, kCtrShards * sizeof(DevCounters), hipMemcpyDeviceToHost);
     DevCounters h{};
     for(const DevCounters& d : shards) { h.rank_queries += d.rank_queries; h.block_loads += d.block_loads; h.table_loads += d.table_loads; }
     lrsc_kernel_stats& s = ctx->stats[which];
diff --git a/longreadselfcorrect_amd/csrc/dp_deal.h b/longreadselfcorrect_amd/csrc/dp_deal.h
--- /dev/null
+++ b/longreadselfcorrect_amd/csrc/dp_deal.h
@@ -0,0 +1,39 @@
+#pragma once
+#include <stdint.h>
+
+#include <algorithm>
+#include <vector>
+
+namespace lrsc {
+
+struct DpDealLaunch {
+    uint64_t work;
+    uint32_t lds;
+};
+
+inline std::vector<std::vector<uint32_t>> dp_deal(const std::vector<DpDealLaunch>& launches, uint32_t n_streams)
+{
+    std::vector<std::vector<uint32_t>> out(n_streams);
+    if(n_streams == 0) return out;
+    std::vector<uint32_t> by_work(launches.size());
+    for(uint32_t i = 0; i < by_work.size(); ++i) by_work[i] = i;
+    std::sort(by_work.begin(), by_work.end(), [&](uint32_t x, uint32_t y) {
+        return launches[x].work != launches[y].work ? launches[x].work > launches[y].work : x < y;
+    });
+    std::vector<uint64_t> load(n_streams, 0);
+    for(uint32_t i : by_work) {
+        uint32_t s = 0;
+        for(uint32_t t = 1; t < n_streams; ++t)
+            if(load[t] < load[s] || (load[t] == load[s] && out[t].size() < out[s].size())) s = t;
+        out[s].push_back(i);
+        const uint64_t w = launches[i].work;
+        load[s] = load[s] > UINT64_MAX - w ? UINT64_MAX : load[s] + w;
+    }
+    for(std::vector<uint32_t>& st : out)
+        std::sort(st.begin(), st.end(), [&](uint32_t x, uint32_t y) {
+            return launches[x].lds != launches[y].lds ? launches[x].lds > launches[y].lds : x < y;
+        });
+    return out;
+}
+
+}
diff --git a/longreadselfcorrect_amd/csrc/dp_dev.h b/longreadselfcorrect_amd/csrc/dp_dev.h
--- a/longreadselfcorrect_amd/csrc/dp_dev.h
+++ b/longreadselfcorrect_amd/csrc/dp_dev.h
@@ -96,10 +96,11 @@
 hipError_t launch_dp_align(const DpAlignArgs& a, uint32_t n_waves, hipStream_t stream);
 hipError_t launch_dp_seeds(const FmIndexDev& fm, const DpPipeArgs& a, hipStream_t stream);
 hipError_t launch_dp_retrieve(const FmIndexDev& fm, const DpPipeArgs& a, hipStream_t stream);
-hipError_t launch_dp_msa(const DpPipeArgs& a, hipStream_t stream);
+hipError_t launch_dp_msa(const DpPipeArgs& a, uint32_t lds_per_cu, hipStream_t stream);
 uint32_t dp_msa_lds_bytes(uint32_t w_cols, uint32_t lq, uint32_t str_cap, uint32_t ops_cap, uint32_t n_str);
 constexpr uint32_t dp_msa_columns(uint32_t lq) { return 3 * lq + 128; }
 constexpr uint32_t dp_cons_capacity(uint32_t lq) { return 2 * lq + 128; }
-uint32_t dp_msa_waves(const DpPipeArgs& a, bool global);
+constexpr uint32_t kLdsPerCu = 160u * 1024u, kLdsGranule = 1280u;
+uint32_t dp_msa_waves(const DpPipeArgs& a, bool global, uint32_t lds_per_cu);
 
 }
diff --git a/longreadselfcorrect_amd/csrc/dp_msa.hip b/longreadselfcorrect_amd/csrc/dp_msa.hip
--- a/longreadselfcorrect_amd/csrc/dp_msa.hip
+++ b/longreadselfcorrect_amd/csrc/dp_msa.hip
@@ -386,33 +386,33 @@
     }
 }
 
-uint32_t dp_msa_waves(const DpPipeArgs& a, bool global)
+uint32_t dp_msa_waves(const DpPipeArgs& a, bool global, uint32_t lds_per_cu)
 {
     int cus = 256, dev = 0;
     (void)hipGetDevice(&dev);
     (void)hipDeviceGetAttribute(&cus, hipDeviceAttributeMultiprocessorCount, dev);
-    uint32_t per_cu = global ? 8u : (a.lds_bytes ? (160u * 1024u) / a.lds_bytes : 16u);
+    uint32_t per_cu = global ? 8u : (a.lds_bytes ? lds_per_cu / a.lds_bytes : 16u);
     per_cu = per_cu < 1 ? 1 : per_cu > 32 ? 32 : per_cu;
     uint32_t n_waves = (uint32_t)cus * per_cu;
     const uint32_t n_work = a.req_list ? a.n_list : a.n_reqs;
     return n_waves > n_work ? n_work : n_waves;
 }
 
-hipError_t launch_dp_msa(const DpPipeArgs& a, hipStream_t stream)
+hipError_t launch_dp_msa(const DpPipeArgs& a, uint32_t lds_per_cu, hipStream_t stream)
 {
     const uint32_t n_work = a.req_list ? a.n_list : a.n_reqs;
     if(n_work == 0) return hipSuccess;
     if(a.msa_ws) {
-        hipLaunchKernelGGL(dp_msa_kernel<true>, dim3(dp_msa_waves(a, true)), dim3(64), 0, stream, a);
+        hipLaunchKernelGGL(dp_msa_kernel<true>, dim3(dp_msa_waves(a, true, lds_per_cu)), dim3(64), 0, stream, a);
         return hipGetLastError();
     }
-    if(a.lds_bytes > 160 * 1024) return hipErrorInvalidValue;
+    if(a.lds_bytes > kLdsPerCu) return hipErrorInvalidValue;
     if(a.lds_bytes > 64 * 1024) {
         const hipError_t e = hipFuncSetAttribute(reinterpret_cast<const void*>(dp_msa_kernel<false>),
                                                  hipFuncAttributeMaxDynamicSharedMemorySize, (int)a.lds_bytes);
         if(e != hipSuccess) return e;
     }
-    hipLaunchKernelGGL(dp_msa_kernel<false>, dim3(dp_msa_waves(a, false)), dim3(64), a.lds_bytes, stream, a);
+    hipLaunchKernelGGL(dp_msa_kernel<false>, dim3(dp_msa_waves(a, false, lds_per_cu)), dim3(64), a.lds_bytes, stream, a);
     return hipGetLastError();
 }
 
diff --git a/longreadselfcorrect_amd/csrc/wp.h b/longreadselfcorrect_amd/csrc/wp.h
--- a/longreadselfcorrect_amd/csrc/wp.h
+++ b/longreadselfcorrect_amd/csrc/wp.h
@@ -188,6 +188,7 @@
 hipError_t launch_wp_begin(const FmIndexDev& fm, const WpArgs& a, hipStream_t stream);
 hipError_t launch_wp_extend(const FmIndexDev& fm, const WpArgs& a, hipStream_t stream);
 hipError_t launch_wp_extend_wave(const FmIndexDev& fm, const WpArgs& a, hipStream_t stream);
+hipError_t wp_extend_wave_static_lds(bool wide, uint32_t* bytes);
 hipError_t launch_wp_wide_collect(const WpArgs& a, uint32_t* out, uint32_t* n_out, hipStream_t stream);
 hipError_t launch_wp_extend_wide(const FmIndexDev& fm, const WpArgs& a, hipStream_t stream);
 hipError_t launch_wp_dp_collect(const WpArgs& a, const WpDpItem* items, hipStream_t stream);
diff --git a/longreadselfcorrect_amd/csrc/wp_wave.hip b/longreadselfcorrect_amd/csrc/wp_wave.hip
--- a/longreadselfcorrect_amd/csrc/wp_wave.hip
+++ b/longreadselfcorrect_amd/csrc/wp_wave.hip
@@ -358,4 +358,13 @@
     return hipGetLastError();
 }
 
-}
+hipError_t wp_extend_wave_static_lds(bool wide, uint32_t* bytes)
+{
+    hipFuncAttributes fa{};
+    const void* f = wide ? reinterpret_cast<const void*>(wp_extend_wave_kernel<true>) : reinterpret_cast<const void*>(wp_extend_wave_kernel<false>);
+    const hipError_t e = hipFuncGetAttributes(&fa, f);
+    if(e == hipSuccess) *bytes = (uint32_t)fa.sharedSizeBytes;
+    return e;
+}
+
+}
```

Result: faster. 148.9, median of 6 (+1.4%).
